# beast-dev/beast-mcmc

Measured on NVIDIA H100. Metric: tree log-likelihood evals/sec, higher is better.
Workload: dtype f64

## Files before the change

beast-mcmc_b200/csrc/api.cu:

```cuda
#include "../../include/libhmsbeagle_b200.h"
#include "engine.h"
#include "multi.h"

#include <algorithm>
#include <atomic>
#include <chrono>
#include <cmath>
#include <cstdio>
#include <cstdlib>
#include <cstring>
#include <string>
#include <unordered_map>

using namespace b200;

namespace {

std::mutex gMutex;
std::vector<Instance*> gInstances;

const long kSupportedFlags =
    BEAGLE_FLAG_PRECISION_DOUBLE | BEAGLE_FLAG_PRECISION_SINGLE | BEAGLE_FLAG_COMPUTATION_SYNCH | BEAGLE_FLAG_EIGEN_REAL |
    BEAGLE_FLAG_EIGEN_COMPLEX | BEAGLE_FLAG_SCALING_MANUAL | BEAGLE_FLAG_SCALING_DYNAMIC |
    BEAGLE_FLAG_SCALERS_RAW | BEAGLE_FLAG_SCALERS_LOG | BEAGLE_FLAG_VECTOR_NONE | BEAGLE_FLAG_THREADING_NONE |
    BEAGLE_FLAG_PROCESSOR_GPU | BEAGLE_FLAG_FRAMEWORK_CUDA | BEAGLE_FLAG_PARALLELOPS_GRID |
    BEAGLE_FLAG_PREORDER_TRANSPOSE_AUTO;

int envInt(const char* name, int dflt) {
    const char* v = getenv(name);
    return v ? atoi(v) : dflt;
}

int flushPending(Instance* in);

Instance* getInstance(int id) {
    std::lock_guard<std::mutex> lock(gMutex);
    if (id < 0 || id >= (int)gInstances.size()) return nullptr;
    return gInstances[id];
}

#define SH(id, expr)                                                                         \
    do {                                                                                     \
        Instance* p__ = getInstance(id);                                                     \
        if (p__ != nullptr && p__->shard != nullptr) {                                       \
            Sharded* sh = static_cast<Sharded*>(p__->shard);                                 \
            (void)sh;                                                                        \
            return (expr);                                                                   \
        }                                                                                    \
    } while (0)

#define GET_INSTANCE_LAZY(in, id)                                       \
    Instance* in = getInstance(id);                                     \
    if (in == nullptr) return BEAGLE_ERROR_UNINITIALIZED_INSTANCE;      \
    if (in->shard != nullptr) return BEAGLE_ERROR_NO_IMPLEMENTATION;    \
    if (cudaSetDevice(in->device) != cudaSuccess) return BEAGLE_ERROR_GENERAL;

#define GET_INSTANCE(in, id)                                            \
    GET_INSTANCE_LAZY(in, id)                                           \
    if (!in->pendingMats.empty() || !in->pendingOps.empty()) {          \
        const int flushRc__ = flushPending(in);                         \
        if (flushRc__ != BEAGLE_SUCCESS) return flushRc__;              \
    }

#define CUDA_OK(expr)                                                                        \
    do {                                                                                     \
        cudaError_t e__ = (expr);                                                            \
        if (e__ != cudaSuccess) {                                                            \
            if (getenv("B200_BEAGLE_DEBUG"))                                                 \
                fprintf(stderr, "[b200-beagle] %s failed: %s (%s:%d)\n", #expr,              \
                        cudaGetErrorString(e__), __FILE__, __LINE__);                        \
            return e__ == cudaErrorMemoryAllocation ? BEAGLE_ERROR_OUT_OF_MEMORY             \
                                                    : BEAGLE_ERROR_GENERAL;                  \
        }                                                                                    \
    } while (0)

struct TimedScope {
    Instance* in;
    int cls;
    cudaEvent_t a = nullptr, b = nullptr;
    TimedScope(Instance* i, int c, int kernels = 1) : in(i), cls(c) {
        if (in->timing) {
            in->timedLaunches[cls] += kernels - 1;
            cudaEventCreate(&a);
            cudaEventCreate(&b);
            cudaEventRecord(a, in->stream);
        }
    }
    ~TimedScope() {
        if (in->timing) {
            cudaEventRecord(b, in->stream);
            in->timed[cls].push_back({a, b});
        }
    }
};

void* stage(Instance* in, const void* src, size_t bytes) {
    size_t need = (bytes + 255) & ~size_t(255);
    if (need > in->stageSize) return nullptr;
    if (in->stagePos + need > in->stageSize) {
        cudaStreamSynchronize(in->stream);
        in->stagePos = 0;
    }
    char* h = in->hStage + in->stagePos;
    char* d = in->dStage + in->stagePos;
    memcpy(h, src, bytes);
    if (cudaMemcpyAsync(d, h, bytes, cudaMemcpyHostToDevice, in->stream) != cudaSuccess) return nullptr;
    in->stagePos += need;
    return d;
}

int uploadSmall(Instance* in, void* dDst, const void* src, size_t bytes) {
    size_t need = (bytes + 255) & ~size_t(255);
    if (need > in->stageSize) return BEAGLE_ERROR_OUT_OF_RANGE;
    if (in->stagePos + need > in->stageSize) {
        cudaStreamSynchronize(in->stream);
        in->stagePos = 0;
    }
    char* h = in->hStage + in->stagePos;
    memcpy(h, src, bytes);
    in->stagePos += need;
    CUDA_OK(cudaMemcpyAsync(dDst, h, bytes, cudaMemcpyHostToDevice, in->stream));
    return BEAGLE_SUCCESS;
}

char* ensurePartials(Instance* in, int idx) {
    if (in->partials[idx] == nullptr) {
        if (in->nextSlot >= in->nSlots) return nullptr;
        in->slotOf[idx] = in->nextSlot++;
        in->partials[idx] = in->partialsBase + (size_t)in->slotOf[idx] * in->partialsElems * in->elemBytes();
    }
    return in->partials[idx];
}

bool validRange(int idx, int n) { return idx >= 0 && idx < n; }

void destroyInstance(Instance* in) {
    if (in->shard != nullptr) { shardedDestroy(in); delete in; return; }
    cudaSetDevice(in->device);
    exchangeRelease(in);
    if (in->stream) cudaStreamSynchronize(in->stream);
    cudaFree(in->partialsBase); cudaFree(in->states8Base); cudaFree(in->states32Base);
    for (CachedPlan& cp : in->planCache) { cp.dropGraph(); cudaFree(cp.dBlock); }
    cudaFree(in->dEigen); cudaFree(in->dMat); cudaFree(in->dEvec); cudaFree(in->dIncSums); cudaFree(in->dIncCounter);
    cudaFree(in->dRecipe);
    if (in->hMapped) cudaFreeHost(in->hMapped); cudaFree(in->dRates); cudaFree(in->dWeights);
    cudaFree(in->dFreqs); cudaFree(in->dScale); cudaFree(in->dPatternWeights);
    cudaFree(in->dPatternPartitions); cudaFree(in->dSite); cudaFree(in->dBlockSums); cudaFree(in->dOut);
    cudaFree(in->dCounter); cudaFree(in->dStage); cudaFree(in->dScratch);
    if (in->hStage) cudaFreeHost(in->hStage);
    if (in->hOut) cudaFreeHost(in->hOut);
    for (int c = 0; c < T_CLASSES; ++c)
        for (auto& ev : in->timed[c]) { cudaEventDestroy(ev.first); cudaEventDestroy(ev.second); }
    if (in->stream) cudaStreamDestroy(in->stream);
    delete in;
}

std::vector<BeagleResource> gResources;
std::vector<int> gShardDevices;
int gShardResource = -1;
std::vector<std::string> gResourceStrings;
BeagleResourceList gResourceList = {nullptr, 0};
std::once_flag gResourceOnce;

void buildResources() {
    int n = 0;
    if (cudaGetDeviceCount(&n) != cudaSuccess) { cudaGetLastError(); n = 0; }
    gResourceStrings.reserve(2 * (n + 1));
    gResourceStrings.push_back("CPU (host)");
    gResourceStrings.push_back("no host implementation in this library | use a GPU resource (1..N)");
    for (int d = 0; d < n; ++d) {
        cudaDeviceProp prop;
        if (cudaGetDeviceProperties(&prop, d) != cudaSuccess) { cudaGetLastError(); continue; }
        char buf[512];
        snprintf(buf, sizeof buf, "%s", prop.name);
        gResourceStrings.push_back(buf);
        snprintf(buf, sizeof buf, "Global memory (MB): %zu | SMs: %d | compute capability: %d.%d | "
                 "native walk kernels (sm_90a), fp64 arithmetic, fp64 or fp32 (4-state) partials",
                 (size_t)(prop.totalGlobalMem >> 20), prop.multiProcessorCount, prop.major, prop.minor);
        gResourceStrings.push_back(buf);
    }
    gShardDevices.clear();
    if (const char* env = getenv("B200_SHARD_DEVICES")) {
        for (const char* q = env; *q;) {
            char* end = nullptr;
            const long d = strtol(q, &end, 10);
            if (end == q) break;
            if (d >= 0 && d < n) gShardDevices.push_back((int)d);
            q = (*end == ',') ? end + 1 : end;
        }
    } else {
        for (int d = 0; d < n; ++d) gShardDevices.push_back(d);
    }
    if (gShardDevices.size() > (size_t)kMaxGroup) gShardDevices.resize(kMaxGroup);
    if (!gShardDevices.empty()) {
        char buf[512];
        snprintf(buf, sizeof buf, "GPU x %zu (pattern-sharded)", gShardDevices.size());
        gResourceStrings.push_back(buf);
        snprintf(buf, sizeof buf, "one instance over %zu GPUs | contiguous pattern blocks (Patterns.java:142-169 rule) | "
                 "per-shard sums added over NVLink inside the root kernel", gShardDevices.size());
        gResourceStrings.push_back(buf);
        gShardResource = (int)(gResourceStrings.size() / 2) - 1;
    }
    size_t count = gResourceStrings.size() / 2;
    gResources.resize(count);
    for (size_t r = 0; r < count; ++r) {
        gResources[r].name = const_cast<char*>(gResourceStrings[2 * r].c_str());
        gResources[r].description = const_cast<char*>(gResourceStrings[2 * r + 1].c_str());
        gResources[r].supportFlags = (r == 0) ? (BEAGLE_FLAG_PROCESSOR_CPU | BEAGLE_FLAG_FRAMEWORK_CPU) : kSupportedFlags;
        gResources[r].requiredFlags = (r == 0) ? BEAGLE_FLAG_FRAMEWORK_CPU : BEAGLE_FLAG_FRAMEWORK_CUDA;
    }
    gResourceList.list = gResources.data();
    gResourceList.length = (int)count;
}

char gImplName[] = "B200-CUDA-Double";
char gImplNameSingle[] = "B200-CUDA-Single";
char gImplDesc[] = "sm_90a walk kernels: one launch per operation list, shared-memory operand stack";


struct Sub { int begin, end, pBase, pLimit; };
struct Plan {
    std::vector<int> order;
    std::vector<Sub> subs;
    std::vector<int> phaseStart;
};

void planPhases(const std::vector<HostOp>& ops, int nBuffers, bool allowReorder, int fixedT, int wantSubs, int minT,
                int smallRemainder, Plan& plan) {
    const int n = (int)ops.size();
    auto single = [&]() {
        plan.order.resize(n);
        for (int k = 0; k < n; ++k) plan.order[k] = k;
        plan.subs.assign(1, Sub{0, n, 0, 0});
        plan.phaseStart = {0, 1};
    };
    if (!allowReorder || n < 2) { single(); return; }
    std::vector<int> writer(nBuffers, -1);
    for (int k = 0; k < n; ++k) {
        if (writer[ops[k].dest] >= 0) { single(); return; }
        writer[ops[k].dest] = k;
    }
    std::vector<int> ch0(n, -1), ch1(n, -1), parent(n, -1);
    for (int k = 0; k < n; ++k) {
        const int a = writer[ops[k].c1], b = writer[ops[k].c2];
        if (a >= 0) { if (a >= k || parent[a] >= 0) { single(); return; } ch0[k] = a; parent[a] = k; }
        if (b >= 0 && ops[k].c2 != ops[k].c1) { if (b >= k || parent[b] >= 0) { single(); return; } ch1[k] = b; parent[b] = k; }
        if (ops[k].dest == ops[k].c1 || ops[k].dest == ops[k].c2) { single(); return; }
    }
    std::vector<char> alive(n, 1);
    std::vector<int> size(n), need(n);
    std::vector<std::pair<int, int>> stack;
    plan.order.clear(); plan.order.reserve(n);
    plan.subs.clear(); plan.phaseStart.assign(1, 0);
    int remaining = n;
    while (remaining > 0) {
        const int T = fixedT > 0 ? fixedT : (remaining <= smallRemainder ? remaining : std::max(minT, (remaining + wantSubs - 1) / wantSubs));
        for (int k = 0; k < n; ++k) {
            if (!alive[k]) continue;
            const int a = (ch0[k] >= 0 && alive[ch0[k]]) ? ch0[k] : -1;
            const int b = (ch1[k] >= 0 && alive[ch1[k]]) ? ch1[k] : -1;
            size[k] = 1 + (a >= 0 ? size[a] : 0) + (b >= 0 ? size[b] : 0);
            int na = a >= 0 ? need[a] : 0, nb = b >= 0 ? need[b] : 0;
            if (na < nb) std::swap(na, nb);
            need[k] = std::max(1, std::max(na, nb + (nb > 0 ? 1 : 0)));
        }
        for (int r = 0; r < n; ++r) {
            if (!alive[r] || size[r] > T) continue;
            if (parent[r] >= 0 && size[parent[r]] <= T) continue;
            const int begin = (int)plan.order.size();
            stack.push_back({r, 0});
            while (!stack.empty()) {
                auto [k, stageNo] = stack.back();
                stack.pop_back();
                if (stageNo == 1) { plan.order.push_back(k); continue; }
                stack.push_back({k, 1});
                const int a = (ch0[k] >= 0 && alive[ch0[k]]) ? ch0[k] : -1;
                const int b = (ch1[k] >= 0 && alive[ch1[k]]) ? ch1[k] : -1;
                const int na = a >= 0 ? need[a] : -1, nb = b >= 0 ? need[b] : -1;
                if (na >= nb) { if (b >= 0) stack.push_back({b, 0}); if (a >= 0) stack.push_back({a, 0}); }
                else          { if (a >= 0) stack.push_back({a, 0}); if (b >= 0) stack.push_back({b, 0}); }
            }
            plan.subs.push_back(Sub{begin, (int)plan.order.size(), 0, 0});
        }
        for (int q = plan.subs[plan.phaseStart.back()].begin; q < (int)plan.order.size(); ++q) alive[plan.order[q]] = 0;
        std::stable_sort(plan.subs.begin() + plan.phaseStart.back(), plan.subs.end(),
                         [](const Sub& a, const Sub& b) { return (a.end - a.begin) > (b.end - b.begin); });
        remaining = n - (int)plan.order.size();
        plan.phaseStart.push_back((int)plan.subs.size());
    }
}

void planLevels(const std::vector<HostOp>& ops, int nBuffers, Plan& plan) {
    const int n = (int)ops.size();
    std::vector<int> writer(nBuffers, -1), level(n, 0);
    bool hazard = false;
    for (int k = 0; k < n; ++k) { if (writer[ops[k].dest] >= 0) hazard = true; writer[ops[k].dest] = k; }
    int maxLevel = 0;
    for (int k = 0; k < n && !hazard; ++k) {
        for (int src : {ops[k].c1, ops[k].c2}) {
            const int w = writer[src];
            if (w < 0) continue;
            if (w >= k) { hazard = true; break; }
            level[k] = std::max(level[k], level[w] + 1);
        }
        maxLevel = std::max(maxLevel, level[k]);
    }
    plan.order.resize(n);
    for (int k = 0; k < n; ++k) plan.order[k] = k;
    plan.subs.clear();
    if (hazard) { plan.subs.assign(1, Sub{0, n, 0, 0}); plan.phaseStart = {0, 1}; return; }
    std::stable_sort(plan.order.begin(), plan.order.end(), [&](int a, int b) { return level[a] < level[b]; });
    plan.phaseStart.assign(1, 0);
    for (int pos = 0; pos < n; ++pos) {
        if (pos > 0 && level[plan.order[pos]] != level[plan.order[pos - 1]]) plan.phaseStart.push_back((int)plan.subs.size());
        plan.subs.push_back(Sub{pos, pos + 1, 0, 0});
    }
    plan.phaseStart.push_back((int)plan.subs.size());
}

void planPreorderPhases(const std::vector<HostOp>& ops, int nBuffers, int fixedT, int wantSubs, int minT,
                        int smallRemainder, Plan& plan) {
    const int n = (int)ops.size();
    std::vector<int> writer(nBuffers, -1), parent(n, -1);
    bool ok = n >= 2;
    for (int k = 0; k < n && ok; ++k) { ok = writer[ops[k].dest] < 0; writer[ops[k].dest] = k; }
    for (int k = 0; k < n && ok; ++k) {
        const int a = writer[ops[k].c1];
        ok = writer[ops[k].c2] < 0 && (a < 0 || a < k) && ops[k].dest != ops[k].c1 && ops[k].dest != ops[k].c2;
        parent[k] = a;
    }
    if (!ok) { planLevels(ops, nBuffers, plan); return; }
    std::vector<std::vector<int>> kids(n);
    for (int k = 0; k < n; ++k) if (parent[k] >= 0) kids[parent[k]].push_back(k);
    std::vector<char> alive(n, 1);
    std::vector<int> size(n), stack;
    std::vector<std::vector<int>> phases;
    int remaining = n;
    while (remaining > 0) {
        const int T = fixedT > 0 ? fixedT : (remaining <= smallRemainder ? remaining : std::max(minT, (remaining + wantSubs - 1) / wantSubs));
        for (int k = n - 1; k >= 0; --k) {
            if (!alive[k]) continue;
            size[k] = 1;
            for (int c : kids[k]) if (alive[c]) size[k] += size[c];
        }
        std::vector<int> roots;
        for (int r = 0; r < n; ++r)
            if (alive[r] && size[r] <= T && !(parent[r] >= 0 && alive[parent[r]] && size[parent[r]] <= T)) roots.push_back(r);
        for (int r : roots) {
            stack.assign(1, r);
            while (!stack.empty()) {
                const int k = stack.back(); stack.pop_back();
                if (!alive[k]) continue;
                alive[k] = 0; --remaining;
                for (int c : kids[k]) if (alive[c]) stack.push_back(c);
            }
        }
        phases.push_back(std::move(roots));
    }
    std::vector<int> phaseOf(n, -1), rootOf(n, -1);
    for (int ph = 0; ph < (int)phases.size(); ++ph)
        for (int r : phases[ph]) { phaseOf[r] = ph; rootOf[r] = r; }
    for (int k = 0; k < n; ++k)
        if (rootOf[k] < 0) { rootOf[k] = rootOf[parent[k]]; phaseOf[k] = phaseOf[parent[k]]; }
    plan.order.clear(); plan.order.reserve(n);
    plan.subs.clear(); plan.phaseStart.assign(1, 0);
    for (int ph = (int)phases.size() - 1; ph >= 0; --ph) {
        for (int r : phases[ph]) {
            const int begin = (int)plan.order.size();
            stack.assign(1, r);
            while (!stack.empty()) {
                const int k = stack.back(); stack.pop_back();
                plan.order.push_back(k);
                for (int q = (int)kids[k].size() - 1; q >= 0; --q)
                    if (rootOf[kids[k][q]] == r) stack.push_back(kids[k][q]);
            }
            plan.subs.push_back(Sub{begin, (int)plan.order.size(), 0, 0});
        }
        std::stable_sort(plan.subs.begin() + plan.phaseStart.back(), plan.subs.end(),
                         [](const Sub& a, const Sub& b) { return (a.end - a.begin) > (b.end - b.begin); });
        plan.phaseStart.push_back((int)plan.subs.size());
    }
}

cudaError_t launchPlan(Instance* in, const void* dOps, const void* dSubs, const std::vector<int>& phaseStart,
                       const std::vector<int>& phaseDepth, bool fourPath, int maxWindow, bool preOrder, int eigenSlot = -1,
                       bool aligned = false, const void* dSnap = nullptr, int nSnap = 0, const void* dVirtTips = nullptr) {
    const bool virt = dVirtTips != nullptr;
    cudaError_t e = cudaSuccess;
    if (nSnap > 0) {
        TimedScope ts(in, T_PARTIALS);
        e = launchCherrySnapshot(in, static_cast<const int4*>(dSnap), nSnap);
    }
    for (size_t ph = 0; ph + 1 < phaseStart.size() && e == cudaSuccess; ++ph) {
        const int s0 = phaseStart[ph], s1 = phaseStart[ph + 1];
        if (s1 <= s0) continue;
        TimedScope ts(in, T_PARTIALS);
        if (fourPath && eigenSlot >= 0 && !preOrder && (ph >= phaseDepth.size() || phaseDepth[ph] == 0)) {
            e = launchWalk4E(in, static_cast<const Op4*>(dOps), static_cast<const int4*>(dSubs) + s0, s1 - s0, maxWindow,
                             aligned, in->hEigen.data() + (size_t)eigenSlot * 36, static_cast<const int4*>(dVirtTips));
            continue;
        }
        if (virt) return cudaErrorInvalidValue;
        e = fourPath ? launchWalk4(in, static_cast<const Op4*>(dOps), static_cast<const int4*>(dSubs) + s0, s1 - s0,
                                   ph < phaseDepth.size() ? phaseDepth[ph] : 0, maxWindow, preOrder)
                     : launchWalkGeneric(in, static_cast<const DevOp*>(dOps), static_cast<const int4*>(dSubs) + s0, s1 - s0,
                                         maxWindow, preOrder);
    }
    return e;
}

cudaError_t accumulateInList(Instance* in, const std::vector<CumGroup>& groups) {
    for (const CumGroup& g : groups) {
        int* dIdx = static_cast<int*>(stage(in, g.indices.data(), sizeof(int) * g.indices.size()));
        if (dIdx == nullptr) return cudaErrorMemoryAllocation;
        cudaError_t e = launchScaleAccumulate(in, dIdx, (int)g.indices.size(), in->dScale + (size_t)g.cum * in->Ppad, 1.0,
                                              g.pBegin, g.pEnd);
        if (e != cudaSuccess) return e;
        in->scaleIsLog[g.cum] = 1;
    }
    return cudaSuccess;
}

void noteScaleWrites(Instance* in, const std::vector<HostOp>& hops) {
    for (const HostOp& o : hops) if (o.sw >= 0) in->scaleIsLog[o.sw] = in->logScalers ? 1 : 0;
}


cudaError_t storeCherries(Instance* in, const int* bufs, int count) {
    if (in->cherryTip1.empty()) return cudaSuccess;
    std::vector<int4> items;
    for (int k = 0; k < count; ++k) {
        const int b = bufs[k];
        if (!validRange(b, in->nBuffers) || in->cherryTip1[b] < 0 || in->cherryStored[b]) continue;
        items.push_back(make_int4(in->slotOf[b], b, in->cherryTip1[b], in->cherryTip2[b]));
        in->cherryStored[b] = 1;
    }
    if (items.empty()) return cudaSuccess;
    const int4* dItems = static_cast<const int4*>(stage(in, items.data(), sizeof(int4) * items.size()));
    cudaError_t e = cudaErrorMemoryAllocation;
    if (dItems != nullptr) {
        TimedScope ts(in, T_PARTIALS);
        e = launchCherryStore(in, dItems, (int)items.size());
    }
    if (e != cudaSuccess) for (const int4& it : items) in->cherryStored[it.y] = 0;
    return e;
}

cudaError_t storeExternal(Instance* in, const std::vector<CherryRef>& external) {
    std::vector<int> bufs;
    for (const CherryRef& x : external) if (x.tip1 < 0) bufs.push_back(x.buf);
    return storeCherries(in, bufs.data(), (int)bufs.size());
}

cudaError_t settleCherriesOf(Instance* in, int t) {
    std::vector<int> deps;
    for (int b = 0; b < (int)in->cherryTip1.size(); ++b)
        if (in->cherryTip1[b] >= 0 && (in->cherryTip1[b] == t || in->cherryTip2[b] == t)) deps.push_back(b);
    const cudaError_t e = storeCherries(in, deps.data(), (int)deps.size());
    if (e == cudaSuccess) for (int b : deps) in->cherryTip1[b] = -1;
    return e;
}

void noteCherryWrites(Instance* in, const std::vector<HostOp>& hops, const std::vector<CherryRef>& cherries) {
    if (in->cherryTip1.empty()) return;
    for (const HostOp& o : hops) in->cherryTip1[o.dest] = -1;
    for (const CherryRef& c : cherries) {
        in->cherryTip1[c.buf] = c.tip1; in->cherryTip2[c.buf] = c.tip2; in->cherryStored[c.buf] = 0;
    }
}

int prepareOps(Instance* in, const std::vector<HostOp>& hops, bool byPartition) {
    for (const HostOp& o : hops) {
        if (!validRange(o.dest, in->nBuffers) || !validRange(o.c1, in->nBuffers) ||
            !validRange(o.c2, in->nBuffers) || !validRange(o.m1, in->nMatrices) ||
            !validRange(o.m2, in->nMatrices))
            return BEAGLE_ERROR_OUT_OF_RANGE;
        if (o.sw != BEAGLE_OP_NONE && !validRange(o.sw, in->nScale)) return BEAGLE_ERROR_OUT_OF_RANGE;
        if (o.sr != BEAGLE_OP_NONE && !validRange(o.sr, in->nScale)) return BEAGLE_ERROR_OUT_OF_RANGE;
        if (o.cum != BEAGLE_OP_NONE && !validRange(o.cum, in->nScale)) return BEAGLE_ERROR_OUT_OF_RANGE;
        if (byPartition && !validRange(o.part, in->partitionCount)) return BEAGLE_ERROR_OUT_OF_RANGE;
    }
    {
        std::vector<char> written(in->nBuffers, 0);
        for (const HostOp& o : hops) written[o.dest] = 1;
        auto holdsData = [&](int b) { return written[b] || in->partials[b] != nullptr || in->states32[b] != nullptr; };
        for (const HostOp& o : hops) {
            if (!holdsData(o.c1) || !holdsData(o.c2)) return BEAGLE_ERROR_OUT_OF_RANGE;
            if (o.kind == 1 && !written[o.c1] && in->states32[o.c1] != nullptr) return BEAGLE_ERROR_OUT_OF_RANGE;
        }
    }
    for (const HostOp& o : hops) {
        if (ensurePartials(in, o.dest) == nullptr) return BEAGLE_ERROR_OUT_OF_MEMORY;
        if (in->states32[o.dest] != nullptr) in->bufferEpoch++;
        in->states8[o.dest] = nullptr;
        in->states32[o.dest] = nullptr;
    }
    return BEAGLE_SUCCESS;
}

int eigenFormSlot(const Instance* in, const std::vector<HostOp>& hops) {
    if (!in->eigenWalk || in->matCP == 0 || in->walkVariant != 0 || hops.empty() || hops[0].kind == 1) return -1;
    const int E = in->matEigen[hops[0].m1];
    if (E < 0 || !in->eigenReal[E]) return -1;
    const unsigned gen = in->eigenGen[E];
    for (const HostOp& o : hops)
        if (in->matEigen[o.m1] != E || in->matEigen[o.m2] != E || in->matEigenGen[o.m1] != gen || in->matEigenGen[o.m2] != gen)
            return -1;
    return E;
}

int planAndLaunch(Instance* in, const std::vector<HostOp>& hops, bool byPartition) {
    const int n = (int)hops.size();
    if (n == 0) return BEAGLE_SUCCESS;
    static_assert(sizeof(HostOp) == 10 * sizeof(int), "HostOp is compared bytewise");
    if (in->planCacheSize > 0) {
        for (CachedPlan& cp : in->planCache) {
            if (cp.dBlock == nullptr || cp.n != n || cp.byPartition != byPartition || cp.epoch != in->bufferEpoch ||
                memcmp(cp.key.data(), hops.data(), sizeof(HostOp) * (size_t)n) != 0)
                continue;
            const int eigenSlot = cp.fourPath ? eigenFormSlot(in, hops) : -1;
            bool stale = cp.readsVirtual && eigenSlot < 0;
            for (const CherryRef& x : cp.external)
                stale = stale || (x.tip1 >= 0 && (in->cherryTip1[x.buf] != x.tip1 || in->cherryTip2[x.buf] != x.tip2));
            if (stale) { cp.dropGraph(); cp.n = -1; continue; }
            CUDA_OK(storeExternal(in, cp.external));
            cp.lastUse = ++in->planClock;
            cp.hits++;
            const unsigned eigenGenNow = eigenSlot >= 0 ? in->eigenGen[eigenSlot] : 0u;
            const void* dSnap = static_cast<char*>(cp.dBlock) + cp.snapOffset;
            const int nSnap = (int)cp.cherries.size();
            const void* dTips = cp.readsVirtual ? static_cast<char*>(cp.dBlock) + cp.tipsOffset : nullptr;
            if (cp.graphExec != nullptr && (cp.graphEigen != eigenSlot || cp.graphEigenGen != eigenGenNow)) {
                if (cp.graphAllEigen && eigenSlot >= 0 && cp.graphEigen == eigenSlot &&
                    updateWalk4EGraph(cp.graphExec, cp.graphKernelNodes, in->hEigen.data() + (size_t)eigenSlot * 36) == cudaSuccess) {
                    cp.graphEigenGen = eigenGenNow;
                } else {
                    cudaGetLastError();
                    cp.dropGraph();
                    cp.hits = 1;
                    if (++cp.graphInvalidations >= 4) cp.graphFailed = true;
                }
            }
            int launches = nSnap > 0;
            for (size_t ph = 0; ph + 1 < cp.phaseStart.size(); ++ph) launches += cp.phaseStart[ph + 1] > cp.phaseStart[ph];
            if (in->useGraphs && launches >= 2 && cp.cumGroups.empty()) {
                if (cp.graphExec == nullptr && !cp.graphFailed && cp.hits >= 2 && !in->timing &&
                    cudaStreamBeginCapture(in->stream, cudaStreamCaptureModeThreadLocal) == cudaSuccess) {
                    const cudaError_t e1 = launchPlan(in, cp.dBlock, static_cast<char*>(cp.dBlock) + cp.subsOffset, cp.phaseStart,
                                                      cp.phaseDepth, cp.fourPath, cp.maxWindow, cp.preOrder, eigenSlot,
                                                      !cp.byPartition, dSnap, nSnap, dTips);
                    cp.graphEigen = eigenSlot;
                    cp.graphEigenGen = eigenGenNow;
                    cudaGraph_t g = nullptr;
                    const cudaError_t e2 = cudaStreamEndCapture(in->stream, &g);
                    if (e1 != cudaSuccess || e2 != cudaSuccess || g == nullptr ||
                        cudaGraphInstantiate(&cp.graphExec, g, 0) != cudaSuccess) {
                        cp.graphExec = nullptr;
                        cp.graphFailed = true;
                        if (g) cudaGraphDestroy(g);
                    } else {
                        cp.graph = g;
                        cp.graphKernelNodes.clear();
                        cp.graphAllEigen = cp.fourPath && eigenSlot >= 0 && !cp.preOrder;
                        for (int dpt : cp.phaseDepth) cp.graphAllEigen = cp.graphAllEigen && dpt == 0;
                        size_t nn = 0;
                        if (cudaGraphGetNodes(g, nullptr, &nn) == cudaSuccess && nn > 0) {
                            std::vector<cudaGraphNode_t> nodes(nn);
                            cudaGraphNodeType ty;
                            if (cudaGraphGetNodes(g, nodes.data(), &nn) == cudaSuccess)
                                for (size_t q = 0; q < nn; ++q)
                                    if (cudaGraphNodeGetType(nodes[q], &ty) == cudaSuccess && ty == cudaGraphNodeTypeKernel)
                                        cp.graphKernelNodes.push_back(nodes[q]);
                        }
                        if (cp.graphKernelNodes.empty()) cp.graphAllEigen = false;
                    }
                    if (getenv("B200_BEAGLE_DEBUG"))
                        fprintf(stderr, "[b200-beagle] graph %s: %d launches\n", cp.graphExec ? "captured" : "capture failed",
                                launches);
                    cudaGetLastError();
                }
                if (cp.graphExec != nullptr) {
                    TimedScope ts(in, T_PARTIALS, launches);
                    CUDA_OK(cudaGraphLaunch(cp.graphExec, in->stream));
                    noteScaleWrites(in, hops);
                    noteCherryWrites(in, hops, cp.cherries);
                    return BEAGLE_SUCCESS;
                }
            }
            CUDA_OK(launchPlan(in, cp.dBlock, static_cast<char*>(cp.dBlock) + cp.subsOffset, cp.phaseStart, cp.phaseDepth,
                               cp.fourPath, cp.maxWindow, cp.preOrder, eigenSlot, !cp.byPartition, dSnap, nSnap,
                               dTips));
            CUDA_OK(accumulateInList(in, cp.cumGroups));
            noteScaleWrites(in, hops);
            noteCherryWrites(in, hops, cp.cherries);
            return BEAGLE_SUCCESS;
        }
    }
    {
        const int rcPrepare = prepareOps(in, hops, byPartition);
        if (rcPrepare != BEAGLE_SUCCESS) return rcPrepare;
    }
    const bool fourState = in->matCP > 0;
    const bool preOrder = hops[0].kind == 1;
    const int eigenSlot = fourState ? eigenFormSlot(in, hops) : -1;
    std::vector<char> written(in->nBuffers, 0);
    std::vector<int> firstWrite(in->nBuffers, n);
    for (int k = n - 1; k >= 0; --k) { written[hops[k].dest] = 1; firstWrite[hops[k].dest] = k; }
    std::vector<CherryRef> cherries;
    std::vector<int4> snap;
    std::vector<HostOp> kept;
    bool readsVirtual = false;
    if (!in->cherryTip1.empty() && !byPartition && !preOrder && eigenSlot >= 0 && !in->stackTail) {
        std::vector<int> writes(in->nBuffers, 0), firstRead(in->nBuffers, n);
        for (int k = 0; k < n; ++k) {
            writes[hops[k].dest]++;
            firstRead[hops[k].c1] = std::min(firstRead[hops[k].c1], k);
            firstRead[hops[k].c2] = std::min(firstRead[hops[k].c2], k);
        }
        for (int k = 0; k < n; ++k) {
            const HostOp& o = hops[k];
            if (in->states8[o.c1] != nullptr && in->states8[o.c2] != nullptr && o.sw == BEAGLE_OP_NONE &&
                o.sr == BEAGLE_OP_NONE && o.cum == BEAGLE_OP_NONE && writes[o.dest] == 1 && firstRead[o.dest] > k) {
                cherries.push_back(CherryRef{o.dest, o.c1, o.c2});
                snap.push_back(make_int4(o.dest, o.m1, o.m2, 0));
            } else {
                kept.push_back(o);
            }
        }
        if (kept.empty()) { cherries.clear(); snap.clear(); }
        readsVirtual = !cherries.empty();
        for (const HostOp& o : hops)
            for (int c : {o.c1, o.c2})
                readsVirtual = readsVirtual || (!written[c] && in->states32[c] == nullptr && in->cherryTip1[c] >= 0);
    }
    Plan plan;
    int maxWindow = in->Ppad;
    const int patsPerWarp = !fourState ? 16 : (in->walkVariant == 2 ? 8 * in->tensorR : (32 / in->matCP) * in->walkR);
    const int warpsPerSM = fourState ? 32 : 12;
    auto wantSubsFor = [&](int window) {
        const int warpsPerSub = std::max(1, (window + patsPerWarp - 1) / patsPerWarp);
        const int over = in->phaseOversub > 0 ? in->phaseOversub : (warpsPerSub >= 32 ? 1 : 2);
        return std::max(1, over * ((in->smCount * warpsPerSM + warpsPerSub - 1) / warpsPerSub));
    };
    if (!byPartition && !preOrder) {
        planPhases(cherries.empty() ? hops : kept, in->nBuffers, in->reorder != 0, in->phaseT, wantSubsFor(in->Ppad),
                   in->phaseTmin, in->phaseSmall, plan);
        bool served = true;
        for (size_t ph = 0; readsVirtual && ph + 1 < plan.phaseStart.size(); ++ph) {
            const int nSubs = plan.phaseStart[ph + 1] - plan.phaseStart[ph];
            served = served && (nSubs == 0 || walk4pServes(in, nSubs, in->Ppad));
        }
        if (!served) {
            readsVirtual = false;
            if (!cherries.empty()) {
                cherries.clear(); snap.clear(); kept.clear();
                planPhases(hops, in->nBuffers, in->reorder != 0, in->phaseT, wantSubsFor(in->Ppad), in->phaseTmin,
                           in->phaseSmall, plan);
            }
        }
        for (Sub& sb : plan.subs) { sb.pBase = 0; sb.pLimit = in->Ppad; }
    }
    const std::vector<HostOp>& L = cherries.empty() ? hops : kept;
    const int nL = (int)L.size();
    std::vector<int> vt1(readsVirtual ? in->nBuffers : 0, -1), vt2(readsVirtual ? in->nBuffers : 0, -1);
    for (const CherryRef& c : cherries) { vt1[c.buf] = c.tip1; vt2[c.buf] = c.tip2; }
    std::vector<CherryRef> external;
    {
        std::vector<char> seen(in->nBuffers, 0);
        for (int k = 0; k < n; ++k)
            for (int c : {hops[k].c1, hops[k].c2}) {
                if (firstWrite[c] < k || in->states32[c] != nullptr || seen[c]) continue;
                seen[c] = 1;
                const bool virt = readsVirtual && !written[c] && in->cherryTip1[c] >= 0;
                external.push_back(CherryRef{c, virt ? in->cherryTip1[c] : -1, virt ? in->cherryTip2[c] : -1});
                if (virt) { vt1[c] = in->cherryTip1[c]; vt2[c] = in->cherryTip2[c]; }
            }
    }
    CUDA_OK(storeExternal(in, external));
    {
        if (!byPartition) {
            if (preOrder) {
                if (in->prePhases) planPreorderPhases(hops, in->nBuffers, in->phaseT, wantSubsFor(in->Ppad), in->phaseTmin, in->phaseSmall, plan);
                else planLevels(hops, in->nBuffers, plan);
                for (Sub& sb : plan.subs) { sb.pBase = 0; sb.pLimit = in->Ppad; }
            }
        } else {
            std::vector<std::vector<int>> members(in->partitionCount);
            for (int k = 0; k < n; ++k) members[hops[k].part].push_back(k);
            std::vector<Plan> plans;
            std::vector<int> base;
            maxWindow = 1;
            for (int part = 0; part < in->partitionCount; ++part) {
                if (members[part].empty()) continue;
                std::vector<HostOp> sub(members[part].size());
                for (size_t q = 0; q < sub.size(); ++q) sub[q] = hops[members[part][q]];
                Plan pl;
                const int window = in->partEnd[part] - in->partBegin[part];
                if (sub[0].kind == 1 && in->prePhases) planPreorderPhases(sub, in->nBuffers, in->phaseT, wantSubsFor(std::max(1, window)), in->phaseTmin, in->phaseSmall, pl);
                else if (sub[0].kind == 1) planLevels(sub, in->nBuffers, pl);
                else planPhases(sub, in->nBuffers, in->reorder != 0, in->phaseT, wantSubsFor(std::max(1, window)), in->phaseTmin, in->phaseSmall, pl);
                base.push_back((int)plan.order.size());
                for (int idx : pl.order) plan.order.push_back(members[part][idx]);
                for (Sub& sb : pl.subs) {
                    sb.begin += base.back(); sb.end += base.back();
                    sb.pBase = in->partBegin[part]; sb.pLimit = in->partEnd[part];
                }
                maxWindow = std::max(maxWindow, window);
                plans.push_back(std::move(pl));
            }
            plan.phaseStart.assign(1, 0);
            for (size_t ph = 0;; ++ph) {
                bool any = false;
                for (const Plan& pl : plans) {
                    if (ph + 1 >= pl.phaseStart.size()) continue;
                    any = true;
                    for (int q = pl.phaseStart[ph]; q < pl.phaseStart[ph + 1]; ++q) plan.subs.push_back(pl.subs[q]);
                }
                if (!any) break;
                plan.phaseStart.push_back((int)plan.subs.size());
            }
        }
    }
    const std::vector<int>& order = plan.order;

    const bool stackEverywhere = fourState && in->walkVariant == 1 && !preOrder;
    const bool stackThin = fourState && in->walkVariant == 0 && in->stackTail && !preOrder;
    const int maxDepth = (stackEverywhere || stackThin) ? in->stackDepthMax : 0;
    const int nPhases = (int)plan.phaseStart.size() - 1;
// ... 208 lines not shown
        if (slot->capacity < blockBytes) {
            if (slot->dBlock) cudaFree(slot->dBlock);
            slot->dBlock = nullptr; slot->capacity = 0;
            if (cudaMalloc(&slot->dBlock, blockBytes) == cudaSuccess) slot->capacity = blockBytes; else cudaGetLastError();
        }
        if (slot->dBlock != nullptr &&
            cudaMemcpyAsync(slot->dBlock, dOps, blockBytes, cudaMemcpyDeviceToDevice, in->stream) == cudaSuccess) {
            slot->key = hops; slot->n = n; slot->byPartition = byPartition; slot->epoch = in->bufferEpoch;
            slot->subsOffset = subsOffset; slot->snapOffset = snapOffset; slot->tipsOffset = tipsOffset;
            slot->cherries = cherries; slot->external = external; slot->readsVirtual = readsVirtual;
            slot->phaseStart = plan.phaseStart; slot->phaseDepth = depths;
            slot->fourPath = fourPath; slot->maxWindow = maxWindow; slot->preOrder = preOrder;
            slot->lastUse = ++in->planClock;
            slot->cumGroups = cumGroups;
            slot->graphFailed = !cumGroups.empty();
        } else if (slot->dBlock != nullptr) {
            slot->n = -1;
        }
    }
    if (tmp != nullptr) { cudaStreamSynchronize(in->stream); cudaFree(tmp); }
    CUDA_OK(e);
    return BEAGLE_SUCCESS;
}

}

namespace b200 {
Instance* instanceById(int id) { return getInstance(id); }
}

extern "C" {

#ifndef B200_SOURCE_HASH
#define B200_SOURCE_HASH "unhashed"
#endif
const char* beagleGetVersion(void) { return "4.0.1-b200+" B200_SOURCE_HASH; }
const char* b200GetSourceHash(void) { return B200_SOURCE_HASH; }

const char* beagleGetCitation(void) {
    return "H100-native tree-likelihood engine exposing the BEAGLE API.\n"
           "API after: Ayres et al. (2019) BEAGLE 3. Syst Biol 68:1052-1061.";
}

BeagleResourceList* beagleGetResourceList(void) {
    std::call_once(gResourceOnce, buildResources);
    return &gResourceList;
}

BeagleBenchmarkedResourceList* beagleGetBenchmarkedResourceList(
    int tipCount, int compactBufferCount, int stateCount, int patternCount, int categoryCount, int* resourceList,
    int resourceCount, long preferenceFlags, long requirementFlags, int eigenModelCount, int partitionCount,
    int calculateDerivatives, long benchmarkFlags);

int beagleCreateInstance(int tipCount, int partialsBufferCount, int compactBufferCount, int stateCount,
                         int patternCount, int eigenBufferCount, int matrixBufferCount, int categoryCount,
                         int scaleBufferCount, int* resourceList, int resourceCount, long preferenceFlags,
                         long requirementFlags, BeagleInstanceDetails* returnInfo) {
    if (tipCount < 0 || partialsBufferCount < 0 || compactBufferCount < 0 || stateCount < 2 ||
        patternCount < 1 || eigenBufferCount < 0 || matrixBufferCount < 0 || categoryCount < 1 ||
        scaleBufferCount < 0 || stateCount > 255)
        return BEAGLE_ERROR_OUT_OF_RANGE;
    if (requirementFlags & ~kSupportedFlags) return BEAGLE_ERROR_NO_RESOURCE;
    const bool singleFits = stateCount <= 4 && categoryCount <= 8;
    if (requirementFlags & BEAGLE_FLAG_PRECISION_SINGLE) {
        if (!singleFits || (requirementFlags & BEAGLE_FLAG_PRECISION_DOUBLE)) return BEAGLE_ERROR_NO_RESOURCE;
    }
    const bool single = singleFits && ((requirementFlags & BEAGLE_FLAG_PRECISION_SINGLE) ||
                                       ((preferenceFlags & BEAGLE_FLAG_PRECISION_SINGLE) &&
                                        !((preferenceFlags | requirementFlags) & BEAGLE_FLAG_PRECISION_DOUBLE)));
    BeagleResourceList* rl = beagleGetResourceList();
    int resource = -1;
    if (resourceList == nullptr || resourceCount <= 0) {
        if (rl->length > 1) resource = 1;
    } else {
        for (int k = 0; k < resourceCount; ++k)
            if (resourceList[k] >= 1 && resourceList[k] < rl->length) { resource = resourceList[k]; break; }
    }
    if (resource < 1) return BEAGLE_ERROR_NO_RESOURCE;

    if (resource == gShardResource) {
        Instance* parent = new Instance();
        parent->resource = resource;
        parent->device = gShardDevices[0];
        parent->P = patternCount; parent->S = stateCount; parent->C = categoryCount; parent->tipCount = tipCount;
        const int g = (int)gShardDevices.size();
        const int rc = shardedCreate(parent, g, gShardDevices.data(), tipCount, partialsBufferCount, compactBufferCount,
                                     stateCount, patternCount, eigenBufferCount, matrixBufferCount, categoryCount,
                                     scaleBufferCount, preferenceFlags, requirementFlags, returnInfo);
        if (rc != BEAGLE_SUCCESS) { delete parent; return rc; }
        if (returnInfo != nullptr) {
            returnInfo->resourceNumber = resource;
            returnInfo->resourceName = rl->list[resource].name;
            parent->flags = returnInfo->flags;
        }
        std::lock_guard<std::mutex> lock(gMutex);
        int id = -1;
        for (size_t k = 0; k < gInstances.size(); ++k) if (gInstances[k] == nullptr) { id = (int)k; break; }
        if (id < 0) { gInstances.push_back(nullptr); id = (int)gInstances.size() - 1; }
        gInstances[id] = parent;
        parent->id = id;
        return id;
    }

    Instance* in = new Instance();
    in->device = resource - 1;
    in->resource = resource;
    if (cudaSetDevice(in->device) != cudaSuccess) { delete in; return BEAGLE_ERROR_NO_RESOURCE; }
    in->tipCount = tipCount; in->nPartials = partialsBufferCount; in->nCompact = compactBufferCount;
    in->S = stateCount; in->P = patternCount; in->nEigen = eigenBufferCount; in->nMatrices = matrixBufferCount;
    in->C = categoryCount; in->nScale = scaleBufferCount;
    in->Sp = stateCount <= 4 ? 4 : ((stateCount + 7) / 8) * 8;
    in->Ppad = ((patternCount + 31) / 32) * 32;
    in->nBuffers = partialsBufferCount + compactBufferCount;
    in->nSets = std::max(1, eigenBufferCount);
    in->single = single;
    in->complexEigen = (requirementFlags | preferenceFlags) & BEAGLE_FLAG_EIGEN_COMPLEX;
    in->logScalers = (requirementFlags | preferenceFlags) & BEAGLE_FLAG_SCALERS_LOG;
    in->flags = (single ? BEAGLE_FLAG_PRECISION_SINGLE : BEAGLE_FLAG_PRECISION_DOUBLE) | BEAGLE_FLAG_COMPUTATION_SYNCH |
                BEAGLE_FLAG_SCALING_MANUAL |
                BEAGLE_FLAG_VECTOR_NONE | BEAGLE_FLAG_THREADING_NONE | BEAGLE_FLAG_PROCESSOR_GPU |
                BEAGLE_FLAG_FRAMEWORK_CUDA | BEAGLE_FLAG_PARALLELOPS_GRID |
                (in->complexEigen ? BEAGLE_FLAG_EIGEN_COMPLEX : BEAGLE_FLAG_EIGEN_REAL) |
                (in->logScalers ? BEAGLE_FLAG_SCALERS_LOG : BEAGLE_FLAG_SCALERS_RAW);
    if ((requirementFlags | preferenceFlags) & BEAGLE_FLAG_PREORDER_TRANSPOSE_AUTO) in->flags |= BEAGLE_FLAG_PREORDER_TRANSPOSE_AUTO;
    if ((requirementFlags | preferenceFlags) & BEAGLE_FLAG_SCALING_DYNAMIC) {
        in->flags &= ~BEAGLE_FLAG_SCALING_MANUAL;
        in->flags |= BEAGLE_FLAG_SCALING_DYNAMIC;
    }
    in->partialsElems = (size_t)in->C * in->Ppad * in->Sp;
    if (in->Sp == 4 && in->C <= 32) {
        int cp = 1;
        while (cp < in->C) cp <<= 1;
        in->matCP = cp;
        in->matStride = (size_t)16 * cp + 52 * (size_t)in->C;
        in->matStride = (in->matStride + 3) & ~size_t(3);
    } else {
        in->matCP = 0;
        in->matStride = (size_t)in->C * in->Sp * (in->Sp + 2 * (size_t)(in->Sp + 4));
    }
    in->slotOf.assign(in->nBuffers, -1);
    in->partials.assign(in->nBuffers, nullptr);
    in->states8.assign(in->nBuffers, nullptr);
    in->states32.assign(in->nBuffers, nullptr);
    in->scaleIsLog.assign(std::max(1, in->nScale), in->logScalers ? 1 : 0);
    in->matEigen.assign(std::max(1, in->nMatrices), -1);
    in->matEigenGen.assign(std::max(1, in->nMatrices), 0u);
    in->eigenGen.assign(std::max(1, in->nEigen), 0u);
    in->eigenReal.assign(std::max(1, in->nEigen), 0);
    in->hEigen.assign((size_t)std::max(1, in->nEigen) * 36, 0.0);
    in->eigenWalk = envInt("B200_EIGEN_WALK", 1);
    in->tipMode = envInt("B200_TIP_MODE", 3);
    in->thinTipMode = envInt("B200_THIN_TIP_MODE", in->tipMode);
    in->virtualCherries = envInt("B200_VIRTUAL_CHERRIES", 1);
    in->walkBlock = 128;
    in->walkVariant = envInt("B200_WALK_VARIANT", 0);
    in->reorder = envInt("B200_REORDER", 1);
    in->forward = envInt("B200_FORWARD", 1);
    in->lookahead = envInt("B200_LOOKAHEAD", 1);
    in->useGraphs = envInt("B200_GRAPHS", 1);
    in->prePhases = envInt("B200_PRE_PHASES", 1);
    in->lookaheadPre = envInt("B200_LOOKAHEAD_PRE", 1);
    in->planCacheSize = std::max(0, std::min(16, envInt("B200_PLAN_CACHE", 4)));
    in->planCache.reserve(16);
    in->thinR1 = envInt("B200_THIN_R1", 1);
    in->stackTail = envInt("B200_STACK_TAIL", 0);
    in->phaseT = envInt("B200_PHASE_T", 0);
    in->phaseTmin = std::max(1, envInt("B200_PHASE_TMIN", 4));
    in->phaseSmall = envInt("B200_PHASE_SMALL", 24);
    in->phaseOversub = std::max(0, envInt("B200_PHASE_OVERSUB", 0));
    in->walkMinBlocks = envInt("B200_WALK_MINB", 4);
    in->walkMinBlocksSet = getenv("B200_WALK_MINB") != nullptr;
    in->tensorR = envInt("B200_TENSOR_R", 2) >= 4 ? 4 : 2;
    in->genericMma = envInt("B200_GENERIC_MMA", 1);
    in->mmaWarps = envInt("B200_MMA_WARPS", 4) == 8 ? 8 : 4;
    cudaDeviceProp prop;
    bool ok = cudaGetDeviceProperties(&prop, in->device) == cudaSuccess;
    if (ok) { in->smCount = prop.multiProcessorCount; in->maxSmemOptin = prop.sharedMemPerBlockOptin; }
    in->walkR = envInt("B200_WALK_R", 4);
    if (in->walkR != 1 && in->walkR != 2 && in->walkR != 4 && in->walkR != 8) in->walkR = 4;
    if (getenv("B200_WALK_R") == nullptr && in->matCP > 0) {
        const int G = 32 / in->matCP;
        while (in->walkR > 1 && (in->Ppad + G * in->walkR - 1) / (G * in->walkR) < in->smCount) in->walkR >>= 1;
    }
    in->stackDepthMax = std::min(64, std::max(0, envInt("B200_STACK_DEPTH", 12)));
    if (single) { in->walkVariant = 0; in->stackTail = 0; }

    ok = ok && cudaStreamCreateWithFlags(&in->stream, cudaStreamNonBlocking) == cudaSuccess;
    const size_t eigenStride = 2 * (size_t)in->S * in->S + 2 * in->S;
    const size_t matElems = (size_t)in->nMatrices * in->matStride;
    const int rootBlocks = (in->Ppad + 255) / 256;
    in->stageSize = size_t(8) << 20;
    auto alloc = [&](auto** p, size_t elems) {
        if (!ok) return;
        using T = std::remove_pointer_t<std::remove_pointer_t<decltype(p)>>;
        size_t bytes = std::max<size_t>(elems, 1) * sizeof(T);
        ok = cudaMalloc(reinterpret_cast<void**>(p), bytes) == cudaSuccess &&
             cudaMemsetAsync(*p, 0, bytes, in->stream) == cudaSuccess;
    };
    alloc(&in->dEigen, std::max(1, in->nEigen) * eigenStride);
    alloc(&in->dMat, matElems);
    if (in->matCP > 0) alloc(&in->dEvec, (size_t)in->nMatrices * in->matCP * 4);
    if (in->matCP > 0 && in->matCP <= 8 && in->virtualCherries) {
        alloc(&in->dRecipe, (size_t)in->nBuffers * 32 * in->matCP);
        in->cherryTip1.assign(in->nBuffers, -1);
        in->cherryTip2.assign(in->nBuffers, -1);
        in->cherryStored.assign(in->nBuffers, 0);
    }
    if (in->matCP > 0 && in->matCP <= 8) {
        alloc(&in->dIncSums, (size_t)in->Ppad / 4 + 8);
        alloc(&in->dIncCounter, 4);
        in->fuseSmall = envInt("B200_FUSE", 1);
        if (ok && in->fuseSmall) {
            if (cudaHostAlloc(reinterpret_cast<void**>(&in->hMapped), 64, cudaHostAllocMapped) == cudaSuccess &&
                cudaHostGetDevicePointer(reinterpret_cast<void**>(&in->dMapped), in->hMapped, 0) == cudaSuccess) {
                memset(in->hMapped, 0, 64);
            } else {
                cudaGetLastError();
                if (in->hMapped) cudaFreeHost(in->hMapped);
                in->hMapped = nullptr;
            }
        }
    }
    alloc(&in->dRates, (size_t)in->nSets * in->C);
    alloc(&in->dWeights, (size_t)in->nSets * in->C);
    alloc(&in->dFreqs, (size_t)in->nSets * in->Sp);
    alloc(&in->dScale, (size_t)in->nScale * in->Ppad);
    alloc(&in->dPatternWeights, in->Ppad);
    alloc(&in->dPatternPartitions, in->Ppad);
    alloc(&in->dSite, in->Ppad);
    alloc(&in->dBlockSums, rootBlocks);
    alloc(&in->dOut, 1024);
    alloc(&in->dCounter, 4);
    alloc(&in->dStage, in->stageSize);
    alloc(&in->states8Base, (size_t)std::max(1, in->tipCount) * in->Ppad);
    alloc(&in->states32Base, (size_t)std::max(1, in->tipCount) * in->Ppad);
    if (ok) {
        int want[2] = {in->nPartials, std::max(1, in->nPartials - std::min(in->nCompact, in->tipCount))};
        for (int attempt = 0; attempt < 2 && in->partialsBase == nullptr; ++attempt) {
            size_t bytes = (size_t)want[attempt] * in->partialsElems * in->elemBytes();
            if (cudaMalloc(reinterpret_cast<void**>(&in->partialsBase), bytes) == cudaSuccess) in->nSlots = want[attempt];
            else { cudaGetLastError(); in->partialsBase = nullptr; }
        }
        if (in->partialsBase == nullptr) { destroyInstance(in); return BEAGLE_ERROR_OUT_OF_MEMORY; }
    }
    ok = ok && cudaMallocHost(reinterpret_cast<void**>(&in->hStage), in->stageSize) == cudaSuccess;
    ok = ok && cudaMallocHost(reinterpret_cast<void**>(&in->hOut), 1024 * sizeof(double)) == cudaSuccess;
    if (ok) {
        in->hRates.assign((size_t)in->nSets * in->C, 1.0);
        in->hWeights.assign((size_t)in->nSets * in->C, 0.0);
        in->hFreqs.assign((size_t)in->nSets * 4, 0.0);
        std::vector<double> ones((size_t)std::max(in->nSets * in->C, in->Ppad), 1.0);
        ok = cudaMemcpyAsync(in->dRates, ones.data(), sizeof(double) * in->nSets * in->C, cudaMemcpyHostToDevice,
                             in->stream) == cudaSuccess;
        std::vector<double> w(in->Ppad, 0.0);
        std::fill(w.begin(), w.begin() + in->P, 1.0);
        ok = ok && cudaMemcpyAsync(in->dPatternWeights, w.data(), sizeof(double) * in->Ppad, cudaMemcpyHostToDevice,
                                   in->stream) == cudaSuccess;
        ok = ok && cudaStreamSynchronize(in->stream) == cudaSuccess;
    }
    if (!ok) {
        cudaError_t e = cudaGetLastError();
        destroyInstance(in);
        return e == cudaErrorMemoryAllocation ? BEAGLE_ERROR_OUT_OF_MEMORY : BEAGLE_ERROR_GENERAL;
    }
    in->partitionCount = 1;
    in->partBegin.assign(1, 0);
    in->partEnd.assign(1, in->P);
    {
        std::lock_guard<std::mutex> lock(gMutex);
        int id = -1;
        for (size_t k = 0; k < gInstances.size(); ++k) if (gInstances[k] == nullptr) { id = (int)k; break; }
        if (id < 0) { gInstances.push_back(nullptr); id = (int)gInstances.size() - 1; }
        gInstances[id] = in;
        in->id = id;
    }
    if (returnInfo != nullptr) {
        returnInfo->resourceNumber = resource;
        returnInfo->resourceName = rl->list[resource].name;
        returnInfo->implName = single ? gImplNameSingle : gImplName;
        returnInfo->implDescription = gImplDesc;
        returnInfo->flags = in->flags;
    }
    return in->id;
}

int beagleFinalizeInstance(int instance) {
    Instance* in = nullptr;
    {
        std::lock_guard<std::mutex> lock(gMutex);
        if (instance < 0 || instance >= (int)gInstances.size() || gInstances[instance] == nullptr)
            return BEAGLE_ERROR_UNINITIALIZED_INSTANCE;
        in = gInstances[instance];
        gInstances[instance] = nullptr;
    }
    destroyInstance(in);
    return BEAGLE_SUCCESS;
}

int beagleFinalize(void) {
    std::vector<Instance*> all;
    {
        std::lock_guard<std::mutex> lock(gMutex);
        all.swap(gInstances);
    }
    for (Instance* in : all) if (in) destroyInstance(in);
    return BEAGLE_SUCCESS;
}

int beagleSetCPUThreadCount(int instance, int) {
    SH(instance, BEAGLE_SUCCESS);
    GET_INSTANCE(in, instance);
    (void)in;
    return BEAGLE_SUCCESS;
}

int beagleSetTipStates(int instance, int tipIndex, const int* inStates) {
    SH(instance, shSetTipStates(sh, tipIndex, inStates));
    GET_INSTANCE(in, instance);
    if (!validRange(tipIndex, in->nBuffers) || inStates == nullptr) return BEAGLE_ERROR_OUT_OF_RANGE;
    std::vector<int> s32(in->Ppad, in->S);
    std::vector<uint8_t> s8(in->Ppad, (uint8_t)in->S);
    for (int p = 0; p < in->P; ++p) {
        int s = inStates[p];
        if (s < 0 || s >= in->S) s = in->S;
        s32[p] = s;
        s8[p] = (uint8_t)s;
    }
    if (tipIndex >= in->tipCount) return BEAGLE_ERROR_OUT_OF_RANGE;
    CUDA_OK(settleCherriesOf(in, tipIndex));
    in->states32[tipIndex] = in->states32Base + (size_t)tipIndex * in->Ppad;
    in->states8[tipIndex] = in->states8Base + (size_t)tipIndex * in->Ppad;
    CUDA_OK(cudaMemcpyAsync(in->states32[tipIndex], s32.data(), sizeof(int) * in->Ppad, cudaMemcpyHostToDevice, in->stream));
    CUDA_OK(cudaMemcpyAsync(in->states8[tipIndex], s8.data(), in->Ppad, cudaMemcpyHostToDevice, in->stream));
    CUDA_OK(cudaStreamSynchronize(in->stream));
    in->bufferEpoch++;
    return BEAGLE_SUCCESS;
}

int beagleGetTipStates(int instance, int tipIndex, int* outStates) {
    SH(instance, shGetTipStates(sh, tipIndex, outStates));
    GET_INSTANCE(in, instance);
    if (!validRange(tipIndex, in->nBuffers) || in->states32[tipIndex] == nullptr) return BEAGLE_ERROR_OUT_OF_RANGE;
    CUDA_OK(cudaMemcpyAsync(outStates, in->states32[tipIndex], sizeof(int) * in->P, cudaMemcpyDeviceToHost, in->stream));
    CUDA_OK(cudaStreamSynchronize(in->stream));
    return BEAGLE_SUCCESS;
}

static int setPartialsImpl(Instance* in, int bufferIndex, const double* inPartials, bool perCategory) {
    if (!validRange(bufferIndex, in->nBuffers) || inPartials == nullptr) return BEAGLE_ERROR_OUT_OF_RANGE;
    char* dst = ensurePartials(in, bufferIndex);
    if (dst == nullptr) return BEAGLE_ERROR_OUT_OF_MEMORY;
    CUDA_OK(settleCherriesOf(in, bufferIndex));
    if (!in->cherryTip1.empty()) in->cherryTip1[bufferIndex] = -1;
    std::vector<double> tmp(in->partialsElems, 0.0);
    for (int c = 0; c < in->C; ++c)
        for (int p = 0; p < in->Ppad; ++p) {
            double* row = tmp.data() + ((size_t)c * in->Ppad + p) * in->Sp;
            if (p < in->P) {
                const double* src = inPartials + ((size_t)(perCategory ? c : 0) * in->P + p) * in->S;
// ... 78 lines not shown
int beagleSetEigenDecomposition(int instance, int eigenIndex, const double* inEigenVectors,
                                const double* inInverseEigenVectors, const double* inEigenValues) {
    SH(instance, shBroadcast(sh, [&](int c) { return beagleSetEigenDecomposition(c, eigenIndex, inEigenVectors, inInverseEigenVectors, inEigenValues); }));
    GET_INSTANCE(in, instance);
    if (!validRange(eigenIndex, in->nEigen)) return BEAGLE_ERROR_OUT_OF_RANGE;
    const size_t S = in->S, stride = 2 * S * S + 2 * S;
    std::vector<double> pack(stride, 0.0);
    memcpy(pack.data(), inEigenVectors, sizeof(double) * S * S);
    memcpy(pack.data() + S * S, inInverseEigenVectors, sizeof(double) * S * S);
    memcpy(pack.data() + 2 * S * S, inEigenValues, sizeof(double) * (in->complexEigen ? 2 * S : S));
    if (in->matCP > 0) {
        double h[36] = {0.0};
        for (size_t k = 0; k < S; ++k) h[32 + k] = inEigenValues[k];
        for (size_t i = 0; i < S; ++i)
            for (size_t k = 0; k < S; ++k) { h[4 * i + k] = inEigenVectors[i * S + k]; h[16 + 4 * i + k] = inInverseEigenVectors[i * S + k]; }
        bool real = true;
        if (in->complexEigen) for (size_t k = 0; k < S; ++k) real = real && inEigenValues[S + k] == 0.0;
        double* dst = in->hEigen.data() + (size_t)eigenIndex * 36;
        if (memcmp(dst, h, sizeof h) != 0 || in->eigenGen[eigenIndex] == 0 || (bool)in->eigenReal[eigenIndex] != real) {
            memcpy(dst, h, sizeof h);
            in->eigenGen[eigenIndex]++;
        }
        in->eigenReal[eigenIndex] = real ? 1 : 0;
    }
    return uploadSmall(in, in->dEigen + (size_t)eigenIndex * stride, pack.data(), sizeof(double) * stride);
}

int beagleSetStateFrequencies(int instance, int stateFrequenciesIndex, const double* inStateFrequencies) {
    SH(instance, shBroadcast(sh, [&](int c) { return beagleSetStateFrequencies(c, stateFrequenciesIndex, inStateFrequencies); }));
    GET_INSTANCE(in, instance);
    if (!validRange(stateFrequenciesIndex, in->nSets)) return BEAGLE_ERROR_OUT_OF_RANGE;
    std::vector<double> f(in->Sp, 0.0);
    memcpy(f.data(), inStateFrequencies, sizeof(double) * in->S);
    if (in->hFreqs.size() == (size_t)in->nSets * 4 && in->S <= 4)
        for (int i = 0; i < 4; ++i) in->hFreqs[(size_t)stateFrequenciesIndex * 4 + i] = i < in->S ? inStateFrequencies[i] : 0.0;
    return uploadSmall(in, in->dFreqs + (size_t)stateFrequenciesIndex * in->Sp, f.data(), sizeof(double) * in->Sp);
}

int beagleSetCategoryWeights(int instance, int categoryWeightsIndex, const double* inCategoryWeights) {
    SH(instance, shBroadcast(sh, [&](int c) { return beagleSetCategoryWeights(c, categoryWeightsIndex, inCategoryWeights); }));
    GET_INSTANCE(in, instance);
    if (!validRange(categoryWeightsIndex, in->nSets)) return BEAGLE_ERROR_OUT_OF_RANGE;
    std::copy(inCategoryWeights, inCategoryWeights + in->C, in->hWeights.begin() + (size_t)categoryWeightsIndex * in->C);
    return uploadSmall(in, in->dWeights + (size_t)categoryWeightsIndex * in->C, inCategoryWeights, sizeof(double) * in->C);
}

int beagleSetCategoryRatesWithIndex(int instance, int categoryRatesIndex, const double* inCategoryRates) {
    SH(instance, shBroadcast(sh, [&](int c) { return beagleSetCategoryRatesWithIndex(c, categoryRatesIndex, inCategoryRates); }));
    GET_INSTANCE(in, instance);
    if (!validRange(categoryRatesIndex, in->nSets)) return BEAGLE_ERROR_OUT_OF_RANGE;
    std::copy(inCategoryRates, inCategoryRates + in->C, in->hRates.begin() + (size_t)categoryRatesIndex * in->C);
    return uploadSmall(in, in->dRates + (size_t)categoryRatesIndex * in->C, inCategoryRates, sizeof(double) * in->C);
}

int beagleSetCategoryRates(int instance, const double* inCategoryRates) {
    return beagleSetCategoryRatesWithIndex(instance, 0, inCategoryRates);
}

int beagleSetPatternWeights(int instance, const double* inPatternWeights) {
    SH(instance, shSetPatternWeights(sh, inPatternWeights));
    GET_INSTANCE(in, instance);
    std::vector<double> w(in->Ppad, 0.0);
    memcpy(w.data(), inPatternWeights, sizeof(double) * in->P);
    CUDA_OK(cudaMemcpyAsync(in->dPatternWeights, w.data(), sizeof(double) * in->Ppad, cudaMemcpyHostToDevice, in->stream));
    CUDA_OK(cudaStreamSynchronize(in->stream));
    return BEAGLE_SUCCESS;
}

int beagleSetPatternPartitions(int instance, int partitionCount, const int* inPatternPartitions) {
    SH(instance, BEAGLE_ERROR_NO_IMPLEMENTATION);
    GET_INSTANCE(in, instance);
    if (partitionCount < 1 || partitionCount > 1000) return BEAGLE_ERROR_OUT_OF_RANGE;
    std::vector<int> begin(partitionCount, 0), end(partitionCount, 0);
    int prev = -1;
    for (int p = 0; p < in->P; ++p) {
        int k = inPatternPartitions[p];
        if (k < 0 || k >= partitionCount) return BEAGLE_ERROR_OUT_OF_RANGE;
        if (k < prev) return BEAGLE_ERROR_NO_IMPLEMENTATION;
        if (k != prev) { for (int q = prev + 1; q <= k; ++q) begin[q] = end[q] = p; prev = k; }
        end[k] = p + 1;
    }
    for (int q = prev + 1; q < partitionCount; ++q) begin[q] = end[q] = in->P;
    in->bufferEpoch++;
    in->partitionCount = partitionCount;
    in->partBegin = begin;
    in->partEnd = end;
    in->hostPartitions.assign(inPatternPartitions, inPatternPartitions + in->P);
    return BEAGLE_SUCCESS;
}

static int updateMatricesImpl(Instance* in, const int* eigenIndices, int eigenIndexScalar, const int* rateSets,
                              const int* probabilityIndices, const double* edgeLengths, int count) {
    if (count <= 0) return BEAGLE_SUCCESS;
    std::vector<double> block((size_t)count + (3 * (size_t)count + 1) / 2);
    int* pack = reinterpret_cast<int*>(block.data() + count);
    for (int k = 0; k < count; ++k) {
        int e = eigenIndices ? eigenIndices[k] : eigenIndexScalar;
        int r = rateSets ? rateSets[k] : 0;
        if (!validRange(probabilityIndices[k], in->nMatrices) || !validRange(e, in->nEigen) ||
            !validRange(r, in->nSets))
            return BEAGLE_ERROR_OUT_OF_RANGE;
        pack[k] = probabilityIndices[k];
        pack[count + k] = e;
        pack[2 * (size_t)count + k] = r;
    }
    if (in->matCP > 0)
        for (int k = 0; k < count; ++k) {
            const int e = eigenIndices ? eigenIndices[k] : eigenIndexScalar;
            in->matEigen[probabilityIndices[k]] = e;
            in->matEigenGen[probabilityIndices[k]] = in->eigenGen[e];
        }
    memcpy(block.data(), edgeLengths, sizeof(double) * count);
    double* dLen = static_cast<double*>(stage(in, block.data(), sizeof(double) * block.size()));
    if (dLen == nullptr) return BEAGLE_ERROR_OUT_OF_MEMORY;
    int* dIdx = reinterpret_cast<int*>(dLen + count);
    TimedScope ts(in, T_MATRICES);
    CUDA_OK(launchTransitionMatrices(in, dIdx, dIdx + count, dIdx + 2 * (size_t)count, dLen, count));
    return BEAGLE_SUCCESS;
}

}
namespace {
int flushPendingImpl(Instance* in) {
    int rc = BEAGLE_SUCCESS;
    if (!in->pendingMats.empty()) {
        const int n = (int)in->pendingMats.size();
        std::vector<int> eig(n), rate(n), prob(n);
        std::vector<double> len(n);
        for (int k = 0; k < n; ++k) {
            eig[k] = in->pendingMats[k].eigen; rate[k] = in->pendingMats[k].rateSet;
            prob[k] = in->pendingMats[k].prob; len[k] = in->pendingMats[k].len;
        }
        in->pendingMats.clear();
        rc = updateMatricesImpl(in, eig.data(), 0, rate.data(), prob.data(), len.data(), n);
    }
    if (!in->pendingOps.empty()) {
        std::vector<HostOp> hops;
        hops.swap(in->pendingOps);
        const int rc2 = planAndLaunch(in, hops, false);
        if (rc == BEAGLE_SUCCESS) rc = rc2;
    }
    return rc;
}

bool fusionPossible(const Instance* in) {
    return in->fuseSmall && in->matCP > 0 && in->matCP <= 8 && !in->timing && !in->exchangeOn && in->walkVariant == 0 &&
           in->eigenWalk && in->hMapped != nullptr;
}

int launchFused(Instance* in, int E, int wIdx, int fIdx, int cum, double* outSum) {
    IncArgs A;
    memset(&A, 0, sizeof A);
    A.partials = in->partialsBase; A.stride = in->partialsElems; A.states = in->states8Base; A.mats = in->dMat;
    A.evecs = in->dEvec; A.scale = in->dScale; A.matStride = in->matStride;
    A.S = in->S; A.C = in->C; A.Ppad = in->Ppad; A.P = in->P; A.logScalers = in->logScalers ? 1 : 0;
    const double* h = in->hEigen.data() + (size_t)E * 36;
    for (int q = 0; q < 16; ++q) { A.V[q] = h[q]; A.Vi[q] = h[16 + q]; }
    for (int q = 0; q < 4; ++q) A.eval[q] = h[32 + q];
    A.nMats = (int)in->pendingMats.size();
    std::unordered_map<int, int> pendingOf;
    for (int q = 0; q < A.nMats; ++q) {
        A.mat[q] = IncMat{in->pendingMats[q].prob, in->pendingMats[q].rateSet, in->pendingMats[q].len};
        for (int c = 0; c < 8; ++c) A.rate[q][c] = c < in->C ? in->hRates[(size_t)in->pendingMats[q].rateSet * in->C + c] : 0.0;
        pendingOf[in->pendingMats[q].prob] = q;
    }
    A.nOps = (int)in->pendingOps.size();
    {
        std::vector<int> outside;
        for (int k = 0; k < A.nOps; ++k)
            for (int c : {in->pendingOps[k].c1, in->pendingOps[k].c2}) {
                bool written = false;
                for (int w = 0; w < k; ++w) written = written || in->pendingOps[w].dest == c;
                if (!written) outside.push_back(c);
            }
        CUDA_OK(storeCherries(in, outside.data(), (int)outside.size()));
    }
    int prevDest = -1;
    for (int k = 0; k < A.nOps; ++k) {
        const HostOp& o = in->pendingOps[k];
        IncOp& d = A.op[k];
        const bool t1 = in->states32[o.c1] != nullptr, t2 = in->states32[o.c2] != nullptr;
        int c1 = o.c1, c2 = o.c2, m1 = o.m1, m2 = o.m2;
        d.flags = 0;
        if (k > 0 && !t1 && c1 == prevDest) d.flags = 1;
        else if (k > 0 && !t2 && c2 == prevDest) { std::swap(c1, c2); std::swap(m1, m2); d.flags = 1; }
        const bool s1 = in->states32[c1] != nullptr, s2 = in->states32[c2] != nullptr;
        d.dest = in->slotOf[o.dest];
        d.c1 = s1 ? -(c1 + 1) : in->slotOf[c1];
        d.c2 = s2 ? -(c2 + 1) : in->slotOf[c2];
        auto mat = [&](int m) { auto it = pendingOf.find(m); return it == pendingOf.end() ? m : -(it->second + 1); };
        d.m1 = mat(m1); d.m2 = mat(m2);
        d.sw = o.sw; d.sr = o.sw >= 0 ? -1 : o.sr;
        prevDest = o.dest;
    }
    for (int c = 0; c < 8; ++c) A.weights[c] = c < in->C ? in->hWeights[(size_t)wIdx * in->C + c] : 0.0;
    for (int i = 0; i < 4; ++i) A.freqs[i] = in->hFreqs[(size_t)fIdx * 4 + i];
    A.cum = cum == BEAGLE_OP_NONE ? nullptr : in->dScale + (size_t)cum * in->Ppad;
    A.patternWeights = in->dPatternWeights; A.site = in->dSite; A.blockSums = in->dIncSums; A.counter = in->dIncCounter;
    A.out = in->dOut;
    A.hostOut = in->dMapped;
    A.hostFlag = reinterpret_cast<volatile unsigned long long*>(in->dMapped + 1);
    A.seq = ++in->incSeq;
    CUDA_OK(launchIncremental(in, A));
    noteScaleWrites(in, in->pendingOps);
    noteCherryWrites(in, in->pendingOps, {});
    in->pendingMats.clear();
    in->pendingOps.clear();
    in->fusedLaunches++;
    volatile unsigned long long* flag = reinterpret_cast<volatile unsigned long long*>(in->hMapped + 1);
    const auto t0 = std::chrono::steady_clock::now();
    long spins = 0;
    while (*flag != A.seq) {
        if ((++spins & 0xfff) == 0 &&
            std::chrono::duration<double>(std::chrono::steady_clock::now() - t0).count() > 5.0) {
            CUDA_OK(cudaStreamSynchronize(in->stream));
            if (*flag != A.seq) return BEAGLE_ERROR_GENERAL;
        }
    }
    std::atomic_thread_fence(std::memory_order_acquire);
    *outSum = in->hMapped[0];
    return std::isnan(*outSum) ? BEAGLE_ERROR_FLOATING_POINT : BEAGLE_SUCCESS;
}
int flushPending(Instance* in) { return flushPendingImpl(in); }
}
extern "C" {

int beagleUpdateTransitionMatrices(int instance, int eigenIndex, const int* probabilityIndices,
                                   const int* firstDerivativeIndices, const int* secondDerivativeIndices,
                                   const double* edgeLengths, int count) {
    SH(instance, shBroadcast(sh, [&](int c) { return beagleUpdateTransitionMatrices(c, eigenIndex, probabilityIndices, firstDerivativeIndices, secondDerivativeIndices, edgeLengths, count); }));
    GET_INSTANCE_LAZY(in, instance);
    if (firstDerivativeIndices != nullptr || secondDerivativeIndices != nullptr)
        return BEAGLE_ERROR_NO_IMPLEMENTATION;
    bool defer = fusionPossible(in) && count >= 1 && in->pendingOps.empty() &&
                 (int)in->pendingMats.size() + count <= kIncMaxMats && validRange(eigenIndex, in->nEigen) &&
                 in->eigenReal[eigenIndex] && in->eigenGen[eigenIndex] > 0;
    for (int k = 0; k < count && defer; ++k) {
        defer = validRange(probabilityIndices[k], in->nMatrices);
        for (const Instance::PendingMat& pm : in->pendingMats) defer = defer && pm.prob != probabilityIndices[k] && pm.eigen == eigenIndex;
        for (int q = 0; q < k && defer; ++q) defer = probabilityIndices[q] != probabilityIndices[k];
    }
    if (defer) {
        for (int k = 0; k < count; ++k) {
            in->pendingMats.push_back(Instance::PendingMat{probabilityIndices[k], eigenIndex, 0, edgeLengths[k]});
            in->matEigen[probabilityIndices[k]] = eigenIndex;
            in->matEigenGen[probabilityIndices[k]] = in->eigenGen[eigenIndex];
        }
        return BEAGLE_SUCCESS;
    }
    if (!in->pendingMats.empty() || !in->pendingOps.empty()) { const int rc = flushPending(in); if (rc != BEAGLE_SUCCESS) return rc; }
    return updateMatricesImpl(in, nullptr, eigenIndex, nullptr, probabilityIndices, edgeLengths, count);
}

int beagleUpdateTransitionMatricesWithMultipleModels(int instance, const int* eigenIndices,
                                                     const int* categoryRateIndices, const int* probabilityIndices,
                                                     const int* firstDerivativeIndices,
                                                     const int* secondDerivativeIndices, const double* edgeLengths,
                                                     int count) {
    SH(instance, shBroadcast(sh, [&](int c) { return beagleUpdateTransitionMatricesWithMultipleModels(c, eigenIndices, categoryRateIndices, probabilityIndices, firstDerivativeIndices, secondDerivativeIndices, edgeLengths, count); }));
    GET_INSTANCE(in, instance);
    if (firstDerivativeIndices != nullptr || secondDerivativeIndices != nullptr)
        return BEAGLE_ERROR_NO_IMPLEMENTATION;
    return updateMatricesImpl(in, eigenIndices, 0, categoryRateIndices, probabilityIndices, edgeLengths, count);
}

static inline size_t matIndex(const Instance* in, int c, int i, int j) {
    return in->matCP ? ((size_t)j * in->matCP + c) * 4 + i : ((size_t)c * in->Sp + j) * in->Sp + i;
}

int beagleSetTransitionMatrix(int instance, int matrixIndex, const double* inMatrix, double) {
    SH(instance, shBroadcast(sh, [&](int c) { return beagleSetTransitionMatrix(c, matrixIndex, inMatrix, 0.0); }));
    GET_INSTANCE(in, instance);
    if (!validRange(matrixIndex, in->nMatrices)) return BEAGLE_ERROR_OUT_OF_RANGE;
    if (in->matCP > 0) in->matEigen[matrixIndex] = -1;
    const size_t n = in->matStride;
    std::vector<double> t(n, 0.0);
    for (int c = 0; c < in->C; ++c)
        for (int i = 0; i < in->S; ++i)
            for (int j = 0; j < in->S; ++j)
            {
                const double v = inMatrix[((size_t)c * in->S + i) * in->S + j];
                t[matIndex(in, c, i, j)] = v;
                if (in->matCP) {
                    double* mm = t.data() + 16 * in->matCP;
                    mm[(size_t)c * 32 + i * 4 + j] = v;
                    double* mt = mm + (size_t)in->C * 32;
                    mt[(size_t)c * 20 + j * 4 + i] = v;
                    for (int q = 0; q < 4; ++q) {
                        if (in->S < 4) mt[(size_t)c * 20 + in->S * 4 + q] = q < in->S ? 1.0 : 0.0;
                        else mt[(size_t)c * 20 + 16 + q] = 1.0;
                    }
                } else {
                    const size_t ld = (size_t)in->Sp + 4, half = (size_t)in->C * in->Sp * in->Sp;
                    t[half + ((size_t)c * in->Sp + i) * ld + j] = v;
                    t[half + (size_t)in->C * in->Sp * ld + ((size_t)c * in->Sp + j) * ld + i] = v;
                }
            }
    CUDA_OK(cudaMemcpyAsync(in->dMat + matrixIndex * n, t.data(), sizeof(double) * n, cudaMemcpyHostToDevice, in->stream));
    CUDA_OK(cudaStreamSynchronize(in->stream));
    return BEAGLE_SUCCESS;
}

int beagleGetTransitionMatrix(int instance, int matrixIndex, double* outMatrix) {
    SH(instance, shBroadcast(sh, [&](int c) { return beagleGetTransitionMatrix(c, matrixIndex, outMatrix); }));
    GET_INSTANCE(in, instance);
    if (!validRange(matrixIndex, in->nMatrices)) return BEAGLE_ERROR_OUT_OF_RANGE;
    const size_t n = in->matStride;
// ... 677 lines not shown
```

beast-mcmc_b200/csrc/engine.h:

```cpp
#pragma once
#include <cuda_runtime.h>
#include <cstdint>
#include <mutex>
#include <vector>

namespace b200 {

struct alignas(16) DevOp {
    double* dest;
    const double* c1;
    const double* c2;
    const void* s1;
    const void* s2;
    const double* m1;
    const double* m2;
    double* scaleWrite;
    const double* scaleRead;
    double* cumScale;
    int pBegin, pEnd;
    int srcSlot1, srcSlot2;
    int dstSlot;
    int pad_;
};

struct alignas(16) Op4 {
    int dest, c1, c2, m1;
    int m2, sw, sr, cum;
    int pBegin, pEnd;
    unsigned int slots;
    int pad_;
    int pfA, pfB, pfM1, pfM2;
};

struct CherryRef { int buf, tip1, tip2; };

template <typename T> struct EdgeRefT { const T* post; const int* states; const T* pre; const double* D; double len; };
using EdgeRef = EdgeRefT<double>;

struct HostOp { int dest, sw, sr, c1, m1, c2, m2, part, cum; int kind = 0; };
struct CumGroup { int cum, pBegin, pEnd; std::vector<int> indices; };
struct CachedPlan {
    std::vector<HostOp> key;
    std::vector<CumGroup> cumGroups;
    int n = -1;
    bool byPartition = false, fourPath = false, preOrder = false;
    unsigned long epoch = 0;
    void* dBlock = nullptr;
    size_t capacity = 0, subsOffset = 0, snapOffset = 0, tipsOffset = 0;
    std::vector<CherryRef> cherries, external;
    bool readsVirtual = false;
    std::vector<int> phaseStart, phaseDepth;
    int maxWindow = 0;
    long lastUse = 0;
    long hits = 0;
    cudaGraphExec_t graphExec = nullptr;
    bool graphFailed = false;
    int graphEigen = -2;
    unsigned graphEigenGen = 0;
    int graphInvalidations = 0;
    cudaGraph_t graph = nullptr;
    std::vector<cudaGraphNode_t> graphKernelNodes;
    bool graphAllEigen = false;
    void dropGraph() {
        if (graphExec) cudaGraphExecDestroy(graphExec);
        if (graph) cudaGraphDestroy(graph);
        graphExec = nullptr; graph = nullptr; graphKernelNodes.clear(); graphAllEigen = false;
    }
};

enum TimingClass { T_PARTIALS = 0, T_MATRICES = 1, T_ROOT = 2, T_CLASSES = 3 };

constexpr int kIncMaxOps = 64, kIncMaxMats = 8;
struct IncOp { int dest, c1, c2, m1, m2, sw, sr, flags; };
struct IncMat { int prob, rateSet; double len; };
struct IncArgs {
    void* partials; size_t stride; const uint8_t* states; double* mats; double* evecs; double* scale;
    size_t matStride;
    int S, C, Ppad, P, logScalers, nOps, nMats, pad_;
    double V[16], Vi[16], eval[4];
    double weights[8], freqs[4], rate[kIncMaxMats][8];
    const double* cum; const double* patternWeights;
    double* site; double* blockSums; unsigned int* counter; double* out;
    volatile double* hostOut; volatile unsigned long long* hostFlag; unsigned long long seq;
    IncMat mat[kIncMaxMats];
    IncOp op[kIncMaxOps];
};

constexpr int kMaxGroup = 16;
struct ExchangeSlot { double value; unsigned long long seq; };
struct Exchange {
    int rank = 0, size = 1;
    unsigned long long seq = 0;
    long long timeoutCycles = 0;
    ExchangeSlot* peers[kMaxGroup] = {};
};

struct Instance {
    int id = -1, device = 0, resource = 0;
    int tipCount = 0, nPartials = 0, nCompact = 0, S = 0, P = 0, nEigen = 0, nMatrices = 0, C = 0, nScale = 0;
    int Sp = 0, Ppad = 0, nBuffers = 0, nSets = 1;
    long flags = 0;
    bool logScalers = false, complexEigen = false;
    cudaStream_t stream = nullptr;
    int smCount = 132;
    size_t maxSmemOptin = 0;

    bool single = false;
    size_t partialsElems = 0;
    size_t elemBytes() const { return single ? sizeof(float) : sizeof(double); }
    char* partialsBase = nullptr;
    int nSlots = 0, nextSlot = 0;
    std::vector<int> slotOf;
    std::vector<char*> partials;
    uint8_t* states8Base = nullptr;
    int* states32Base = nullptr;
    std::vector<uint8_t*> states8;
    std::vector<int*> states32;
    int matCP = 0;
    size_t matStride = 0;

    double* dEigen = nullptr;
    double* dMat = nullptr;
    double* dEvec = nullptr;
    std::vector<int> matEigen;
    std::vector<unsigned> matEigenGen, eigenGen;
    std::vector<char> eigenReal;
    std::vector<double> hEigen;
    int eigenWalk = 1;
    int tipMode = 2;
    int thinTipMode = 3;
    int virtualCherries = 1;
    std::vector<int> cherryTip1, cherryTip2;
    std::vector<char> cherryStored;
    double* dRecipe = nullptr;
    double* dRates = nullptr;
    std::vector<double> hRates, hWeights, hFreqs;
    double* dWeights = nullptr;
    double* dFreqs = nullptr;
    double* dScale = nullptr;
    std::vector<char> scaleIsLog;
    double* dPatternWeights = nullptr;
    int* dPatternPartitions = nullptr;
    double* dSite = nullptr;
    double* dBlockSums = nullptr;
    double* dOut = nullptr;
    unsigned int* dCounter = nullptr;
    int lookaheadPre = 1;
    int prePhases = 1;
    int useGraphs = 1;
    int lookahead = 1;
    int forward = 1;
    double* dScratch = nullptr;
    size_t scratchDoubles = 0;
    int partitionCount = 1;
    std::vector<int> partBegin, partEnd;
    std::vector<int> hostPartitions;

    char* hStage = nullptr;
    char* dStage = nullptr;
    size_t stageSize = 0, stagePos = 0;
    double* hOut = nullptr;

    int fuseSmall = 1;
    struct PendingMat { int prob, eigen, rateSet; double len; };
    std::vector<PendingMat> pendingMats;
    std::vector<HostOp> pendingOps;
    int pendingCum = -1;
    double* hMapped = nullptr;
    double* dMapped = nullptr;
    double* dIncSums = nullptr;
    unsigned int* dIncCounter = nullptr;
    unsigned long long incSeq = 0;
    long fusedLaunches = 0;

    void* shard = nullptr;
    Exchange exchange;
    ExchangeSlot* dSlots = nullptr;
    std::vector<void*> ipcOpened;
    bool exchangeOn = false;

    bool timing = false;
    std::vector<std::pair<cudaEvent_t, cudaEvent_t>> timed[T_CLASSES];
    double timedMs[T_CLASSES] = {0, 0, 0};
    long timedLaunches[T_CLASSES] = {0, 0, 0};

    size_t walkSmemConfigured = 0, genericSmemConfigured = 0, mmaSmemConfigured[8] = {0, 0, 0, 0, 0, 0, 0, 0};
    int walkBlock = 128;
    int walkVariant = 0;
    std::vector<CachedPlan> planCache;
    int planCacheSize = 4;
    long planClock = 0;
    unsigned long bufferEpoch = 0;
    int reorder = 1;
    int thinR1 = 1;
    int stackTail = 0;
    int stackDepthMax = 12;
    int walkMinBlocks = 4;
    bool walkMinBlocksSet = false;
    int mmaWarps = 4;
    int tensorR = 2;
    int genericMma = 1;
    int walkR = 4;
    int phaseTmin = 4, phaseOversub = 0, phaseSmall = 24;
    int phaseT = 0;
};

struct Sharded;
Instance* instanceById(int id);
void exchangeRelease(Instance* in);
int shardedCreate(Instance* parent, int g, const int* devices, int tipCount, int partialsBufferCount, int compactBufferCount,
                  int stateCount, int patternCount, int eigenBufferCount, int matrixBufferCount, int categoryCount,
                  int scaleBufferCount, long preferenceFlags, long requirementFlags, void* details );
void shardedDestroy(Instance* parent);

cudaError_t launchTransitionMatrices(Instance* in, const int* dProbIdx, const int* dEigenIdx,
                                     const int* dRateSet, const double* dLengths, int count);
cudaError_t launchWalk4(Instance* in, const Op4* dOps, const int4* dSubs, int nSubs, int stackDepth, int maxWindow, bool preOrder);
cudaError_t updateWalk4EGraph(cudaGraphExec_t exec, const std::vector<cudaGraphNode_t>& kernelNodes, const double* eigen);
cudaError_t launchWalk4E(Instance* in, const Op4* dOps, const int4* dSubs, int nSubs, int maxWindow, bool aligned,
                         const double* eigen, const int4* dVirtTips);
bool walk4pServes(const Instance* in, int nSubs, int maxWindow);
cudaError_t launchCherrySnapshot(Instance* in, const int4* dItems, int count);
cudaError_t launchCherryStore(Instance* in, const int4* dItems, int count);
cudaError_t launchWalkGeneric(Instance* in, const DevOp* dOps, const int4* dSubs, int nSubs, int maxWindow, bool preOrder);
size_t edgeDerivativeWorkspace(const Instance* in, int count);
cudaError_t launchEdgeDerivatives(Instance* in, const EdgeRefT<void>* dEdges, int count, const double* weights, double* outPerPattern,
                                  double* outSum, double* outSumSq, double* partial);
int compressSitePatterns(int device, int taxa, int sites, const int* hStates, int* hPatternOfSite, int* hPatterns,
                         double* hWeights, int* hPatternCount);
int crossProductBlocks(const Instance* in, int count);
cudaError_t launchCrossProducts(Instance* in, const EdgeRefT<void>* dEdges, int count, const double* rates,
                                const double* weights, double* scratch);
cudaError_t launchRoot(Instance* in, const void* root, const double* weights, const double* freqs,
                       const double* cumScale, int pBegin, int pEnd, double* dOutSlot, const Exchange* exchange = nullptr);
cudaError_t launchIncremental(Instance* in, const IncArgs& args);
cudaError_t launchCombineMatrices(Instance* in, const int* dFirst, const int* dSecond, const int* dResult, int count, bool multiply);
cudaError_t launchExchangeSum(Instance* in, const double* dVals, int n, double* dOutJoint, const Exchange* exchange);
cudaError_t launchScaleAccumulate(Instance* in, const int* dIdx, int count, double* cum, double sign,
                                  int pBegin, int pEnd);
cudaError_t launchRescalePartialsForGet(Instance* in, double* tmp, const double* cum);

}
```

beast-mcmc_b200/csrc/incr.cu:

```cuda
#include "engine.h"
#include "walk4.cuh"

namespace b200 {

namespace {

__device__ __forceinline__ double absBitsI(double v) {
    return __hiloint2double(__double2hiint(v) & 0x7fffffff, __double2loint(v));
}

template <typename T, int CP>
__device__ __forceinline__ void incrementalBody(const IncArgs& A) {
    constexpr int G = 32 / CP;
    __shared__ double sE[kIncMaxMats][CP][4];
    __shared__ __align__(16) double sP[kIncMaxMats][CP][16];
    __shared__ double red[4];
    __shared__ bool last;
    const int tid = threadIdx.x, lane = tid & 31, wib = tid >> 5;
    const int S = A.S, C = A.C;
    const int c = lane / G;
    const int p = blockIdx.x * (4 * G) + wib * G + (lane % G);
    const bool catValid = c < C;
    const int cc = catValid ? c : 0;
    const bool inRange = p < A.Ppad;
    const int pp = inRange ? p : 0;
    const size_t off0 = ((size_t)cc * A.Ppad + pp) * 4;
    for (int k = 0; k < A.nOps; ++k) {
        const IncOp op = A.op[k];
#pragma unroll
        for (int ch = 0; ch < 2; ++ch) {
            const int child = ch == 0 ? op.c1 : op.c2, m = ch == 0 ? op.m1 : op.m2;
            if (child < 0) {
                if (c == 0) prefetchL1(A.states + (size_t)(-child - 1) * A.Ppad + pp);
                if (m >= 0 && lane < 4) prefetchL1(A.mats + (size_t)m * A.matStride + lane * 4 * CP);
            } else {
                if (!(ch == 0 && (op.flags & 1)) && catValid)
                    prefetchL1(static_cast<const T*>(A.partials) + (size_t)child * A.stride + off0);
                if (m >= 0 && lane == 0) prefetchL1(A.evecs + (size_t)m * CP * 4);
            }
        }
        if (op.sr >= 0 && c == 0) prefetchL1(A.scale + (size_t)op.sr * A.Ppad + pp);
    }
    if (c == 0) {
        prefetchL1(A.patternWeights + pp);
        if (A.cum != nullptr) prefetchL1(A.cum + pp);
    }
    for (int idx = tid; idx < A.nMats * C * 4; idx += 128) {
        const int q = idx / (C * 4), c = (idx >> 2) % C, k = idx & 3;
        sE[q][c][k] = k < S ? exp(A.eval[k] * A.rate[q][c] * A.mat[q].len) : 0.0;
    }
    __syncthreads();
    for (int idx = tid; idx < A.nMats * C * 16; idx += 128) {
        const int q = idx / (C * 16), c = (idx >> 4) % C, j = (idx >> 2) & 3, i = idx & 3;
        double acc = 0.0;
        if (i < S && j < S) {
#pragma unroll
            for (int k = 0; k < 4; ++k) acc += A.V[4 * i + k] * (sE[q][c][k] * A.Vi[4 * k + j]);
            acc = fabs(acc);
        }
        sP[q][c][j * 4 + i] = acc;
        if (blockIdx.x == 0) {
            double* base = A.mats + (size_t)A.mat[q].prob * A.matStride;
            base[((size_t)j * CP + c) * 4 + i] = acc;
            double* mm = base + 16 * CP;
            mm[(size_t)c * 32 + i * 4 + j] = acc;
            mm[(size_t)c * 32 + 16 + i * 4 + j] = 0.0;
            double* mt = mm + (size_t)C * 32;
            mt[(size_t)c * 20 + j * 4 + i] = (j < S) ? acc : ((j == S && i < S) ? 1.0 : 0.0);
            if (j == 0) mt[(size_t)c * 20 + 16 + i] = (S == 4 && i < S) ? 1.0 : 0.0;
            if (j == 0) A.evecs[((size_t)A.mat[q].prob * CP + c) * 4 + i] = sE[q][c][i];
        }
    }
    __syncthreads();

    double d[4] = {0.0, 0.0, 0.0, 0.0};
    for (int k = 0; k < A.nOps; ++k) {
        const IncOp op = A.op[k];
#pragma unroll
        for (int ch = 0; ch < 2; ++ch) {
            const int child = ch == 0 ? op.c1 : op.c2, m = ch == 0 ? op.m1 : op.m2;
            double y[4];
            if (child < 0) {
                const int s = (int)__ldg(A.states + (size_t)(-child - 1) * A.Ppad + pp);
                if (s < S) {
                    if (m < 0) {
                        const double* col = &sP[-m - 1][cc][s * 4];
                        y[0] = col[0]; y[1] = col[1]; y[2] = col[2]; y[3] = col[3];
                    } else {
                        ldg256_ro(A.mats + (size_t)m * A.matStride + ((size_t)s * CP + cc) * 4, y);
                    }
                } else {
#pragma unroll
                    for (int i = 0; i < 4; ++i) y[i] = (i < S) ? 1.0 : 0.0;
                }
            } else {
                double e[4], x[4], u[4];
                if (m < 0) { e[0] = sE[-m - 1][cc][0]; e[1] = sE[-m - 1][cc][1]; e[2] = sE[-m - 1][cc][2]; e[3] = sE[-m - 1][cc][3]; }
                else ldg256_ro(A.evecs + ((size_t)m * CP + cc) * 4, e);
                if (ch == 0 && (op.flags & 1)) {
#pragma unroll
                    for (int i = 0; i < 4; ++i) x[i] = d[i];
                } else {
                    loadCell(static_cast<const T*>(A.partials) + (size_t)child * A.stride + off0, x);
                }
#pragma unroll
                for (int q = 0; q < 4; ++q)
                    u[q] = (A.Vi[4 * q] * x[0] + A.Vi[4 * q + 1] * x[1] + A.Vi[4 * q + 2] * x[2] + A.Vi[4 * q + 3] * x[3]) * e[q];
#pragma unroll
                for (int i = 0; i < 4; ++i)
                    y[i] = absBitsI(A.V[4 * i] * u[0] + A.V[4 * i + 1] * u[1] + A.V[4 * i + 2] * u[2] + A.V[4 * i + 3] * u[3]);
            }
#pragma unroll
            for (int i = 0; i < 4; ++i) d[i] = ch == 0 ? y[i] : d[i] * y[i];
        }
        if (op.sw >= 0) {
            double mx = catValid ? fmax(fmax(d[0], d[1]), fmax(d[2], d[3])) : 0.0;
#pragma unroll
            for (int sh = G; sh < 32; sh <<= 1) mx = fmax(mx, __shfl_xor_sync(0xffffffffu, mx, sh));
            if (mx == 0.0) mx = 1.0;
            const double inv = 1.0 / mx;
#pragma unroll
            for (int i = 0; i < 4; ++i) d[i] *= inv;
            if (c == 0 && inRange) A.scale[(size_t)op.sw * A.Ppad + p] = A.logScalers ? log(mx) : mx;
        } else if (op.sr >= 0) {
            double f = A.scale[(size_t)op.sr * A.Ppad + pp];
            if (A.logScalers) f = exp(f);
            const double inv = 1.0 / f;
#pragma unroll
            for (int i = 0; i < 4; ++i) d[i] *= inv;
        }
        roundCell<T>(d);
        if (catValid && inRange) storeCell(static_cast<T*>(A.partials) + (size_t)op.dest * A.stride + off0, d);
    }

    double t = 0.0;
    if (catValid) t = A.weights[cc] * (A.freqs[0] * d[0] + A.freqs[1] * d[1] + A.freqs[2] * d[2] + A.freqs[3] * d[3]);
#pragma unroll
    for (int sh = G; sh < 32; sh <<= 1) t += __shfl_xor_sync(0xffffffffu, t, sh);
    double contrib = 0.0;
    if (c == 0 && p < A.P) {
        double s = log(t);
        if (A.cum != nullptr) s += A.cum[p];
        A.site[p] = s;
        contrib = A.patternWeights[p] * s;
    }
#pragma unroll
    for (int sh = 16; sh > 0; sh >>= 1) contrib += __shfl_xor_sync(0xffffffffu, contrib, sh);
    if (lane == 0) red[wib] = contrib;
    __syncthreads();
    if (tid == 0) {
        A.blockSums[blockIdx.x] = (red[0] + red[1]) + (red[2] + red[3]);
        __threadfence();
        const unsigned done = atomicAdd(A.counter, 1u);
        last = (done == gridDim.x - 1);
    }
    __syncthreads();
    if (last) {
        __threadfence();
        double acc = 0.0;
        for (int q = tid; q < (int)gridDim.x; q += 128) acc += A.blockSums[q];
#pragma unroll
        for (int sh = 16; sh > 0; sh >>= 1) acc += __shfl_xor_sync(0xffffffffu, acc, sh);
        __syncthreads();
        if (lane == 0) red[wib] = acc;
        __syncthreads();
        if (tid == 0) {
            const double total = (red[0] + red[1]) + (red[2] + red[3]);
            *A.out = total;
            *A.counter = 0u;
            *A.hostOut = total;
            __threadfence_system();
            *A.hostFlag = A.seq;
        }
    }
}

template <int CP>
__global__ void __launch_bounds__(128)
k_incremental(const IncArgs A) {
    incrementalBody<double, CP>(A);
}

template <int CP>
__global__ void __launch_bounds__(128)
k_incrementals(const IncArgs A) {
    incrementalBody<float, CP>(A);
}

}

cudaError_t launchIncremental(Instance* in, const IncArgs& A) {
    const int G = 32 / in->matCP;
    const int blocks = (in->Ppad + 4 * G - 1) / (4 * G);
    if (in->single) {
        switch (in->matCP) {
            case 1: k_incrementals<1><<<blocks, 128, 0, in->stream>>>(A); break;
            case 2: k_incrementals<2><<<blocks, 128, 0, in->stream>>>(A); break;
            case 4: k_incrementals<4><<<blocks, 128, 0, in->stream>>>(A); break;
            case 8: k_incrementals<8><<<blocks, 128, 0, in->stream>>>(A); break;
            default: return cudaErrorInvalidValue;
        }
        return cudaGetLastError();
    }
    switch (in->matCP) {
        case 1: k_incremental<1><<<blocks, 128, 0, in->stream>>>(A); break;
        case 2: k_incremental<2><<<blocks, 128, 0, in->stream>>>(A); break;
        case 4: k_incremental<4><<<blocks, 128, 0, in->stream>>>(A); break;
        case 8: k_incremental<8><<<blocks, 128, 0, in->stream>>>(A); break;
        default: return cudaErrorInvalidValue;
    }
    return cudaGetLastError();
}

}
```

beast-mcmc_b200/csrc/kernels.cu:

```cuda
#include "engine.h"
#include "walk4.cuh"

#include <algorithm>
#include <cfloat>

namespace b200 {

__device__ __forceinline__ void dmma884acc(double& d0, double& d1, double a, double b) {
    asm("mma.sync.aligned.m8n8k4.row.col.f64.f64.f64.f64 {%0,%1}, {%2}, {%3}, {%0,%1};"
        : "+d"(d0), "+d"(d1) : "d"(a), "d"(b));
}

__global__ void k_transition(const double* __restrict__ eigenBase, size_t eigenStride, int S, int Sp, int C,
                             int complexForm, const double* __restrict__ ratesBase,
                             const int* __restrict__ probIdx, const int* __restrict__ eigenIdx,
                             const int* __restrict__ rateSet, const double* __restrict__ lengths,
                             double* __restrict__ matBase, size_t matStride, int matCP, double* __restrict__ evecBase) {
    extern __shared__ double sm[];
    double* ec = sm;
    double* ss = sm + S;
    int* pt = reinterpret_cast<int*>(sm + 2 * S);
    const int b = blockIdx.x, c = blockIdx.y;
    const double* E = eigenBase + (size_t)eigenIdx[b] * eigenStride;
    const double* evec = E;
    const double* ievc = E + (size_t)S * S;
    const double* eval = E + 2 * (size_t)S * S;
    const double d = lengths[b] * ratesBase[(size_t)rateSet[b] * C + c];
    for (int k = threadIdx.x; k < S; k += blockDim.x) {
        double im = complexForm ? eval[S + k] : 0.0;
        if (im == 0.0) {
            ec[k] = exp(d * eval[k]); ss[k] = 0.0; pt[k] = k;
        } else {
            int run = 0;
            for (int q = k - 1; q >= 0 && eval[S + q] != 0.0; --q) ++run;
            const bool first = (run % 2 == 0);
            int k0 = first ? k : k - 1;
            double bb = eval[S + k0];
            double expat = exp(d * eval[k0]);
            ec[k] = expat * cos(d * bb);
            ss[k] = (first ? 1.0 : -1.0) * expat * sin(d * bb);
            pt[k] = first ? k + 1 : k - 1;
        }
    }
    __syncthreads();
    if (evecBase != nullptr && threadIdx.x < 4)
        evecBase[((size_t)probIdx[b] * matCP + c) * 4 + threadIdx.x] = threadIdx.x < S ? ec[threadIdx.x] : 0.0;
    double* out = matBase + (size_t)probIdx[b] * matStride + (matCP ? (size_t)c * 4 : (size_t)c * Sp * Sp);
    const int rowStride = matCP ? matCP * 4 : Sp;
    for (int idx = threadIdx.x; idx < Sp * Sp; idx += blockDim.x) {
        int j = idx / Sp, i = idx % Sp;
        double acc = 0.0;
        if (i < S && j < S) {
            for (int k = 0; k < S; ++k) {
                double iexp = ec[k] * ievc[(size_t)k * S + j] + ss[k] * ievc[(size_t)pt[k] * S + j];
                acc += evec[(size_t)i * S + k] * iexp;
            }
            acc = fabs(acc);
        }
        out[(size_t)j * rowStride + i] = acc;
        if (!matCP) {
            const size_t ld = (size_t)Sp + 4;
            double* padded = matBase + (size_t)probIdx[b] * matStride + (size_t)C * Sp * Sp;
            padded[((size_t)c * Sp + i) * ld + j] = acc;
            padded[(size_t)C * Sp * ld + ((size_t)c * Sp + j) * ld + i] = acc;
        } else {
            double* mm = matBase + (size_t)probIdx[b] * matStride + 16 * matCP;
            mm[(size_t)c * 32 + i * 4 + j] = acc;
            mm[(size_t)c * 32 + 16 + i * 4 + j] = 0.0;
            double* mt = mm + (size_t)C * 32;
            mt[(size_t)c * 20 + j * 4 + i] = (j < S) ? acc : ((j == S && i < S) ? 1.0 : 0.0);
            if (j == 0) mt[(size_t)c * 20 + 16 + i] = (S == 4 && i < S) ? 1.0 : 0.0;
        }
    }
}

__device__ __forceinline__ size_t matEntry(int matCP, int Sp, int c, int i, int j) {
    return matCP ? ((size_t)j * matCP + c) * 4 + i : ((size_t)c * Sp + j) * Sp + i;
}
__global__ void __launch_bounds__(256)
k_combine_matrices(double* __restrict__ matBase, size_t matStride, int S, int Sp, int C, int matCP,
                   const int* __restrict__ first, const int* __restrict__ second, const int* __restrict__ result, int multiply) {
    const int q = blockIdx.x, c = blockIdx.y;
    const double* A = matBase + (size_t)first[q] * matStride;
    const double* B = matBase + (size_t)second[q] * matStride;
    double* R = matBase + (size_t)result[q] * matStride;
    for (int idx = threadIdx.x; idx < Sp * Sp; idx += blockDim.x) {
        const int i = idx / Sp, j = idx % Sp;
        double v = 0.0;
        if (i < S && j < S) {
            if (multiply) for (int k = 0; k < S; ++k) v += A[matEntry(matCP, Sp, c, i, k)] * B[matEntry(matCP, Sp, c, k, j)];
            else v = A[matEntry(matCP, Sp, c, i, j)] + B[matEntry(matCP, Sp, c, i, j)];
        }
        R[matEntry(matCP, Sp, c, i, j)] = v;
        if (!matCP) {
            const size_t ld = (size_t)Sp + 4;
            double* padded = R + (size_t)C * Sp * Sp;
            padded[((size_t)c * Sp + i) * ld + j] = v;
            padded[(size_t)C * Sp * ld + ((size_t)c * Sp + j) * ld + i] = v;
        } else {
            double* mm = R + 16 * matCP;
            mm[(size_t)c * 32 + i * 4 + j] = v;
            mm[(size_t)c * 32 + 16 + i * 4 + j] = 0.0;
            double* mt = mm + (size_t)C * 32;
            mt[(size_t)c * 20 + j * 4 + i] = (j < S) ? v : ((j == S && i < S) ? 1.0 : 0.0);
            if (j == 0) mt[(size_t)c * 20 + 16 + i] = (S == 4 && i < S) ? 1.0 : 0.0;
        }
    }
}

cudaError_t launchCombineMatrices(Instance* in, const int* dFirst, const int* dSecond, const int* dResult, int count, bool multiply) {
    if (count <= 0) return cudaSuccess;
    k_combine_matrices<<<dim3(count, in->C), 256, 0, in->stream>>>(in->dMat, in->matStride, in->S, in->Sp, in->C, in->matCP,
                                                                   dFirst, dSecond, dResult, multiply ? 1 : 0);
    return cudaGetLastError();
}

template <int NT>
__global__ void __launch_bounds__(128)
k_transition_mma(const double* __restrict__ eigenBase, size_t eigenStride, int S, int C,
                 const double* __restrict__ ratesBase, const int* __restrict__ probIdx,
                 const int* __restrict__ eigenIdx, const int* __restrict__ rateSet,
                 const double* __restrict__ lengths, double* __restrict__ matBase, size_t matStride) {
    constexpr int Sp = 8 * NT;
    constexpr int LD = Sp + 4;
    extern __shared__ double smt[];
    double* As = smt;
    double* Bt = smt + Sp * LD;
    double* ex = Bt + Sp * LD;
    const int b = blockIdx.x, c = blockIdx.y, tid = threadIdx.x;
    const double* E = eigenBase + (size_t)eigenIdx[b] * eigenStride;
    const double* evec = E;
    const double* ievc = E + (size_t)S * S;
    const double* eval = E + 2 * (size_t)S * S;
    const double d = lengths[b] * ratesBase[(size_t)rateSet[b] * C + c];
    for (int k = tid; k < Sp; k += 128) ex[k] = k < S ? exp(d * eval[k]) : 0.0;
    __syncthreads();
    for (int q = tid; q < Sp * Sp; q += 128) {
        const int r = q / Sp, col = q % Sp;
        As[r * LD + col] = (r < S && col < S) ? evec[(size_t)r * S + col] : 0.0;
        Bt[col * LD + r] = (r < S && col < S) ? ievc[(size_t)r * S + col] * ex[r] : 0.0;
    }
    __syncthreads();
    const int lane = tid & 31, w = tid >> 5, g = lane >> 2, t = lane & 3;
    double* outT = matBase + (size_t)probIdx[b] * matStride + (size_t)c * Sp * Sp;
    double* outR = matBase + (size_t)probIdx[b] * matStride + (size_t)C * Sp * Sp + (size_t)c * Sp * LD;
    double* outTp = outR + (size_t)C * Sp * LD;
    for (int mt = w; mt < NT; mt += 4) {
        double acc[NT][2];
#pragma unroll
        for (int n = 0; n < NT; ++n) { acc[n][0] = 0.0; acc[n][1] = 0.0; }
        const double* arow = As + (8 * mt + g) * LD + t;
        const double* brow = Bt + g * LD + t;
#pragma unroll 4
        for (int kc = 0; kc < Sp / 4; ++kc) {
            const double a = arow[4 * kc];
#pragma unroll
            for (int n = 0; n < NT; ++n) dmma884acc(acc[n][0], acc[n][1], a, brow[n * 8 * LD + 4 * kc]);
        }
        const int i = 8 * mt + g;
#pragma unroll
        for (int n = 0; n < NT; ++n) {
            const int j = 8 * n + 2 * t;
            const double v0 = fabs(acc[n][0]), v1 = fabs(acc[n][1]);
            *reinterpret_cast<double2*>(outR + (size_t)i * LD + j) = make_double2(v0, v1);
            outT[(size_t)j * Sp + i] = v0;
            outT[(size_t)(j + 1) * Sp + i] = v1;
            outTp[(size_t)j * LD + i] = v0;
            outTp[(size_t)(j + 1) * LD + i] = v1;
        }
    }
}

template <int NT>
static cudaError_t launchTransitionMmaT(Instance* in, const int* dProbIdx, const int* dEigenIdx, const int* dRateSet,
                                        const double* dLengths, int count) {
    constexpr int Sp = 8 * NT;
    const size_t smem = (2 * (size_t)Sp * (Sp + 4) + Sp) * sizeof(double);
    static_assert(Sp <= 64, "shared-memory budget");
    cudaError_t e = cudaFuncSetAttribute(k_transition_mma<NT>, cudaFuncAttributeMaxDynamicSharedMemorySize, (int)smem);
    if (e != cudaSuccess) return e;
    dim3 grid(count, in->C);
    k_transition_mma<NT><<<grid, 128, smem, in->stream>>>(in->dEigen, 2 * (size_t)in->S * in->S + 2 * in->S, in->S, in->C,
                                                          in->dRates, dProbIdx, dEigenIdx, dRateSet, dLengths, in->dMat,
                                                          in->matStride);
    return cudaGetLastError();
}

cudaError_t launchTransitionMatrices(Instance* in, const int* dProbIdx, const int* dEigenIdx,
                                     const int* dRateSet, const double* dLengths, int count) {
    if (count <= 0) return cudaSuccess;
    if (in->genericMma && in->matCP == 0 && !in->complexEigen) {
        switch (in->Sp / 8) {
            case 1: return launchTransitionMmaT<1>(in, dProbIdx, dEigenIdx, dRateSet, dLengths, count);
            case 2: return launchTransitionMmaT<2>(in, dProbIdx, dEigenIdx, dRateSet, dLengths, count);
            case 3: return launchTransitionMmaT<3>(in, dProbIdx, dEigenIdx, dRateSet, dLengths, count);
            case 4: return launchTransitionMmaT<4>(in, dProbIdx, dEigenIdx, dRateSet, dLengths, count);
            case 8: return launchTransitionMmaT<8>(in, dProbIdx, dEigenIdx, dRateSet, dLengths, count);
            default: break;
        }
    }
    size_t smem = (size_t)in->S * (2 * sizeof(double) + sizeof(int)) + 16;
    int threads = in->Sp * in->Sp >= 1024 ? 256 : (in->Sp * in->Sp >= 128 ? 128 : 32);
    dim3 grid(count, in->C);
    k_transition<<<grid, threads, smem, in->stream>>>(in->dEigen, 2 * (size_t)in->S * in->S + 2 * in->S, in->S,
                                                      in->Sp, in->C, in->complexEigen ? 1 : 0, in->dRates,
                                                      dProbIdx, dEigenIdx, dRateSet, dLengths, in->dMat,
                                                      in->matStride, in->matCP, in->matCP ? in->dEvec : nullptr);
    return cudaGetLastError();
}

struct Mat4 { double r[4][4]; };

template <int CP>
__device__ __forceinline__ void loadMat(const double* __restrict__ m, Mat4& M) {
    ldg256_ro(m, M.r[0]); ldg256_ro(m + 4 * CP, M.r[1]); ldg256_ro(m + 8 * CP, M.r[2]); ldg256_ro(m + 12 * CP, M.r[3]);
}

__device__ __forceinline__ void applyMat(const Mat4& M, const double (&x)[4], double (&y)[4]) {
#pragma unroll
    for (int i = 0; i < 4; ++i) y[i] = M.r[0][i] * x[0] + M.r[1][i] * x[1] + M.r[2][i] * x[2] + M.r[3][i] * x[3];
}

template <typename T, int CP, int R, bool STACK, bool FIRST>
__device__ __forceinline__ void childTerm(const WalkArgs& A, int child, int matIdx, int slot, int moff, size_t off0,
                                          int p0, bool catValid, int pBegin, int pEnd, const double2* stackMem,
                                          int nthreads, double (&y)[R][4]) {
    constexpr int G = 32 / CP;
    const int S = A.S;
    const double* m = A.mats + (size_t)matIdx * A.matStride + moff;
    if (child < 0) {
        const uint8_t* t = A.states + (size_t)(-child - 1) * A.Ppad;
#pragma unroll
        for (int r = 0; r < R; ++r) {
            const int p = p0 + r * G;
            const bool active = catValid && p >= pBegin && p < pEnd;
            const int s = active ? (int)__ldg(t + p) : S;
            double v[4];
            if (s < S) ldg256_ro(m + 4 * CP * s, v);
            else {
#pragma unroll
                for (int i = 0; i < 4; ++i) v[i] = (i < S) ? 1.0 : 0.0;
            }
#pragma unroll
            for (int i = 0; i < 4; ++i) y[r][i] = FIRST ? v[i] : y[r][i] * v[i];
        }
    } else {
        Mat4 M;
        loadMat<CP>(m, M);
        const T* xg = static_cast<const T*>(A.partials) + (size_t)child * A.stride + off0;
#pragma unroll
        for (int r = 0; r < R; ++r) {
            const int p = p0 + r * G;
            const bool active = catValid && p >= pBegin && p < pEnd;
            double x[4], v[4];
            if (STACK && slot != 0xFF) {
                double2 lo = stackMem[((slot * R + r) * 2 + 0) * nthreads + threadIdx.x];
                double2 hi = stackMem[((slot * R + r) * 2 + 1) * nthreads + threadIdx.x];
                x[0] = lo.x; x[1] = lo.y; x[2] = hi.x; x[3] = hi.y;
            } else if (active) {
                loadCell(xg + (size_t)r * G * 4, x);
            } else { x[0] = x[1] = x[2] = x[3] = 0.0; }
            applyMat(M, x, v);
#pragma unroll
            for (int i = 0; i < 4; ++i) y[r][i] = FIRST ? v[i] : y[r][i] * v[i];
        }
    }
}

template <typename T, int CP, int R, bool STACK, bool PRE>
__device__ __forceinline__ void walk4Body(const WalkArgs& A) {
    static_assert(sizeof(T) == 8 || !STACK, "the operand-stack variant is built for fp64 partials only");
    constexpr int G = 32 / CP;
    extern __shared__ double2 stackMem[];
    const int lane = threadIdx.x & 31;
    const int warp = (blockIdx.x * blockDim.x + threadIdx.x) >> 5;
    const int c = lane / G;
    const int4 range = __ldg(A.subs + blockIdx.y);
    const int p0 = range.z + warp * (G * R) + (lane % G);
    if (range.z + warp * (G * R) >= range.w) return;
    const bool catValid = c < A.C;
    const int cc = catValid ? c : 0;
    const size_t off0 = ((size_t)cc * A.Ppad + p0) * 4;
    const int moff = cc * 4;
    const int nthreads = blockDim.x;
    const int last = range.y - 1;

    Op4 cur = loadOp(A.ops + range.x);
    double d[R][4];
#pragma unroll
    for (int r = 0; r < R; ++r) d[r][0] = d[r][1] = d[r][2] = d[r][3] = 0.0;
    for (int k = range.x; k <= last; ++k) {
        Op4 nxt;
        if (R == 1) nxt = loadOp(A.ops + min(k + 1, last));
        else if (lane == 0) prefetchL1(A.ops + min(k + 2, last));
        const int s1 = cur.slots & 0xFF, s2 = (cur.slots >> 8) & 0xFF, sd = (cur.slots >> 16) & 0xFF;
        if (!STACK) {
#pragma unroll
            for (int w = 0; w < 2; ++w) {
                const int pf = w == 0 ? cur.pfA : cur.pfB;
                if (pf == 0) continue;
                if (pf & 1) {
                    const uint8_t* t = A.states + (size_t)(pf >> 1) * A.Ppad + p0;
                    if ((lane % G) == 0 && c == 0) prefetchL1(t);
                } else if (catValid) {
                    const T* xg = static_cast<const T*>(A.partials) + (size_t)((pf >> 1) - 1) * A.stride + off0;
#pragma unroll
                    for (int r = 0; r < R; ++r)
                        if (p0 + r * G < A.Ppad) prefetchL1(xg + (size_t)r * G * 4);
                }
            }
            if (lane < 8) {
                const int mi = lane < 4 ? cur.pfM1 : cur.pfM2;
                if (mi >= 0) prefetchL1(A.mats + (size_t)mi * A.matStride + (lane & 3) * 4 * CP);
            }
        }
        if (!PRE) {
            if (!STACK && (cur.pad_ & 2)) {
                Mat4 M;
                loadMat<CP>(A.mats + (size_t)cur.m1 * A.matStride + moff, M);
#pragma unroll
                for (int r = 0; r < R; ++r) {
                    double v[4];
                    applyMat(M, d[r], v);
#pragma unroll
                    for (int i = 0; i < 4; ++i) d[r][i] = v[i];
                }
            } else {
                childTerm<T, CP, R, STACK, true>(A, cur.c1, cur.m1, s1, moff, off0, p0, catValid, cur.pBegin, cur.pEnd, stackMem, nthreads, d);
            }
            childTerm<T, CP, R, STACK, false>(A, cur.c2, cur.m2, s2, moff, off0, p0, catValid, cur.pBegin, cur.pEnd, stackMem, nthreads, d);
        } else {
            double v[R][4];
            childTerm<T, CP, R, false, true>(A, cur.c2, cur.m2, 0xFF, moff, off0, p0, catValid, cur.pBegin, cur.pEnd, stackMem, nthreads, v);
            Mat4 M1;
            loadMat<CP>(A.mats + (size_t)cur.m1 * A.matStride + moff, M1);
            const T* xg = static_cast<const T*>(A.partials) + (size_t)cur.c1 * A.stride + off0;
            const bool fromRegisters = (cur.pad_ & 2) != 0;
#pragma unroll
            for (int r = 0; r < R; ++r) {
                const int p = p0 + r * G;
                double x[4] = {0.0, 0.0, 0.0, 0.0};
                if (fromRegisters) {
#pragma unroll
                    for (int i = 0; i < 4; ++i) x[i] = d[r][i];
                } else if (catValid && p >= cur.pBegin && p < cur.pEnd) loadCell(xg + (size_t)r * G * 4, x);
                double q[4];
#pragma unroll
                for (int i = 0; i < 4; ++i) q[i] = x[i] * v[r][i];
#pragma unroll
                for (int j = 0; j < 4; ++j) d[r][j] = M1.r[j][0] * q[0] + M1.r[j][1] * q[1] + M1.r[j][2] * q[2] + M1.r[j][3] * q[3];
            }
        }
        if (R != 1) nxt = loadOp(A.ops + min(k + 1, last));
        T* dg = static_cast<T*>(A.partials) + (size_t)cur.dest * A.stride + off0;
#pragma unroll
        for (int r = 0; r < R; ++r) {
            const int p = p0 + r * G;
            const bool active = catValid && p >= cur.pBegin && p < cur.pEnd;
            if (cur.sw >= 0) {
                double m = active ? fmax(fmax(d[r][0], d[r][1]), fmax(d[r][2], d[r][3])) : 0.0;
#pragma unroll
                for (int sh = G; sh < 32; sh <<= 1) m = fmax(m, __shfl_xor_sync(0xffffffffu, m, sh));
                if (m == 0.0) m = 1.0;
                const double inv = 1.0 / m;
#pragma unroll
                for (int i = 0; i < 4; ++i) d[r][i] *= inv;
                if (active && c == 0) {
                    A.scale[(size_t)cur.sw * A.Ppad + p] = A.logScalers ? log(m) : m;
                }
                __syncwarp();
            } else if (cur.sr >= 0) {
                double f = active ? A.scale[(size_t)cur.sr * A.Ppad + p] : 1.0;
                if (A.logScalers) f = exp(f);
                const double inv = 1.0 / f;
// ... 1633 lines not shown
```

beast-mcmc_b200/csrc/walk4.cuh:

```cuda
#pragma once
#include "engine.h"

namespace b200 {

__device__ __forceinline__ void ldg256(const double* p, double (&v)[4]) {
    asm volatile("ld.global.v2.f64 {%0,%1}, [%4];\n\tld.global.v2.f64 {%2,%3}, [%4+16];"
                 : "=d"(v[0]), "=d"(v[1]), "=d"(v[2]), "=d"(v[3]) : "l"(p) : "memory");
}
__device__ __forceinline__ void ldg256_nc(const double* p, double (&v)[4]) {
    asm volatile("ld.global.nc.v2.f64 {%0,%1}, [%4];\n\tld.global.nc.v2.f64 {%2,%3}, [%4+16];"
                 : "=d"(v[0]), "=d"(v[1]), "=d"(v[2]), "=d"(v[3]) : "l"(p));
}
__device__ __forceinline__ void stg256(double* p, const double (&v)[4]) {
    asm volatile("st.global.v2.f64 [%0], {%1,%2};\n\tst.global.v2.f64 [%0+16], {%3,%4};"
                 :: "l"(p), "d"(v[0]), "d"(v[1]), "d"(v[2]), "d"(v[3]) : "memory");
}

template <typename T>
__device__ __forceinline__ void roundCell(double (&v)[4]) {
    if constexpr (sizeof(T) == 4) {
#pragma unroll
        for (int i = 0; i < 4; ++i) {
            float f;
            asm("cvt.rn.f32.f64 %0, %1;" : "=f"(f) : "d"(v[i]));
            const unsigned b = __float_as_uint(f);
            v[i] = (double)((b & 0x7f800000u) ? f : __uint_as_float(b & 0x80000000u));
        }
    }
}
__device__ __forceinline__ void loadCell(const double* p, double (&v)[4]) { ldg256(p, v); }
__device__ __forceinline__ void loadCell(const float* p, double (&v)[4]) {
    float f[4];
    asm volatile("ld.global.v4.f32 {%0,%1,%2,%3}, [%4];" : "=f"(f[0]), "=f"(f[1]), "=f"(f[2]), "=f"(f[3]) : "l"(p) : "memory");
#pragma unroll
    for (int i = 0; i < 4; ++i) v[i] = f[i];
}
__device__ __forceinline__ void storeCell(double* p, const double (&v)[4]) { stg256(p, v); }
__device__ __forceinline__ void storeCell(float* p, const double (&v)[4]) {
    asm volatile("st.global.v4.f32 [%0], {%1,%2,%3,%4};"
                 :: "l"(p), "f"((float)v[0]), "f"((float)v[1]), "f"((float)v[2]), "f"((float)v[3]) : "memory");
}

struct WalkArgs {
    const Op4* ops;
    const int4* subs;
    void* partials;
    size_t stride;
    const uint8_t* states;
    const double* mats;
    double* scale;
    int S, C, Ppad, logScalers;
    size_t matStride;
    int matMmaOffset;
    const double* evecs;
    const double* recipes;
    const int4* virtTips;
    double V[16];
    double Vi[16];
};

__device__ __forceinline__ Op4 loadOp(const Op4* p) {
    const int4* q = reinterpret_cast<const int4*>(p);
    int4 a = __ldg(q), b = __ldg(q + 1), c = __ldg(q + 2), d = __ldg(q + 3);
    Op4 o;
    o.dest = a.x; o.c1 = a.y; o.c2 = a.z; o.m1 = a.w;
    o.m2 = b.x; o.sw = b.y; o.sr = b.z; o.cum = b.w;
    o.pBegin = c.x; o.pEnd = c.y; o.slots = (unsigned)c.z; o.pad_ = c.w;
    o.pfA = d.x; o.pfB = d.y; o.pfM1 = d.z; o.pfM2 = d.w;
    return o;
}

__device__ __forceinline__ void prefetchL1(const void* p) {
    asm volatile("prefetch.global.L1 [%0];" :: "l"(p));
}

__device__ __forceinline__ void ldg256_ro(const double* p, double (&v)[4]) {
    asm("ld.global.nc.v2.f64 {%0,%1}, [%4];\n\tld.global.nc.v2.f64 {%2,%3}, [%4+16];"
        : "=d"(v[0]), "=d"(v[1]), "=d"(v[2]), "=d"(v[3]) : "l"(p));
}
__device__ __forceinline__ void loadCellRo(const double* p, double (&v)[4]) { ldg256_ro(p, v); }
__device__ __forceinline__ void loadCellRo(const float* p, double (&v)[4]) {
    float f[4];
    asm("ld.global.nc.v4.f32 {%0,%1,%2,%3}, [%4];" : "=f"(f[0]), "=f"(f[1]), "=f"(f[2]), "=f"(f[3]) : "l"(p));
#pragma unroll
    for (int i = 0; i < 4; ++i) v[i] = f[i];
}

}
```

beast-mcmc_b200/csrc/walk4e.cu:

```cuda
#include "engine.h"
#include "walk4.cuh"

namespace b200 {

namespace {

__device__ __forceinline__ double absBits(double v) {
    return __hiloint2double(__double2hiint(v) & 0x7fffffff, __double2loint(v));
}

template <typename T, int CP, int R, bool ALIGNED, bool FIRST, int TIP>
__device__ __forceinline__ void childTermE(const WalkArgs& A, const double (&Vi)[16], int child, int matIdx, bool fromRegisters,
                                           int cc, size_t off0, int p0, bool catValid, int pBegin, int pEnd, double (&d)[R][4],
                                           double* tab) {
    constexpr int G = 32 / CP;
    const int S = A.S;
    const bool tip = child < 0;
    if (TIP == 2 && tip) {
        const int lane = threadIdx.x & 31;
        const uint8_t* t = A.states + (size_t)(-child - 1) * A.Ppad;
        int s[R];
#pragma unroll
        for (int r = 0; r < R; ++r) {
            const int p = p0 + r * G;
            s[r] = (ALIGNED || (catValid && p >= pBegin && p < pEnd)) ? (int)__ldg(t + p) : 4;
        }
        const double* m = A.mats + (size_t)matIdx * A.matStride;
        __syncwarp();
#pragma unroll
        for (int q = lane; q < 5 * CP; q += 32) {
            const int c = q / 5, sym = q - 5 * c;
            double v[4];
            if (sym < S && sym < 4 && c < A.C) ldg256_ro(m + (sym * CP + c) * 4, v);
            else {
#pragma unroll
                for (int i = 0; i < 4; ++i) v[i] = (i < S) ? 1.0 : 0.0;
            }
            double2* dst = reinterpret_cast<double2*>(tab + q * 4);
            dst[0] = make_double2(v[0], v[1]);
            dst[1] = make_double2(v[2], v[3]);
        }
        __syncwarp();
#pragma unroll
        for (int r = 0; r < R; ++r) {
            const double2* col = reinterpret_cast<const double2*>(tab + (cc * 5 + min(s[r], 4)) * 4);
            const double2 lo = col[0], hi = col[1];
            if (FIRST) { d[r][0] = lo.x; d[r][1] = lo.y; d[r][2] = hi.x; d[r][3] = hi.y; }
            else { d[r][0] *= lo.x; d[r][1] *= lo.y; d[r][2] *= hi.x; d[r][3] *= hi.y; }
        }
        return;
    }
    if (TIP == 1 && tip) {
        const uint8_t* t = A.states + (size_t)(-child - 1) * A.Ppad;
        const double* m = A.mats + (size_t)matIdx * A.matStride + cc * 4;
#pragma unroll
        for (int r = 0; r < R; ++r) {
            const int p = p0 + r * G;
            const int s = (ALIGNED || (catValid && p >= pBegin && p < pEnd)) ? (int)__ldg(t + p) : S;
            double v[4];
            if (s < S) ldg256_ro(m + 4 * CP * s, v);
            else {
#pragma unroll
                for (int i = 0; i < 4; ++i) v[i] = (i < S) ? 1.0 : 0.0;
            }
#pragma unroll
            for (int i = 0; i < 4; ++i) d[r][i] = FIRST ? v[i] : d[r][i] * v[i];
        }
        return;
    }
    double e[4];
    ldg256_ro(A.evecs + ((size_t)matIdx * CP + cc) * 4, e);
    const uint8_t* t = A.states + (size_t)(tip ? -child - 1 : 0) * A.Ppad;
    const T* xg = static_cast<const T*>(A.partials) + (size_t)(tip ? 0 : child) * A.stride + off0;
#pragma unroll
    for (int r = 0; r < R; ++r) {
        const int p = p0 + r * G;
        const bool live = ALIGNED || (catValid && p >= pBegin && p < pEnd);
        double x[4], u[4], y[4];
        int s = 0;
        if (tip) {
            s = live ? (int)__ldg(t + p) : S;
#pragma unroll
            for (int j = 0; j < 4; ++j) x[j] = (s == j) ? 1.0 : 0.0;
        } else if (fromRegisters) {
#pragma unroll
            for (int i = 0; i < 4; ++i) x[i] = d[r][i];
        } else if (live) {
            loadCell(xg + (size_t)r * G * 4, x);
        } else {
            x[0] = x[1] = x[2] = x[3] = 0.0;
        }
#pragma unroll
        for (int k = 0; k < 4; ++k)
            u[k] = (Vi[4 * k] * x[0] + Vi[4 * k + 1] * x[1] + Vi[4 * k + 2] * x[2] + Vi[4 * k + 3] * x[3]) * e[k];
#pragma unroll
        for (int i = 0; i < 4; ++i)
            y[i] = absBits(A.V[4 * i] * u[0] + A.V[4 * i + 1] * u[1] + A.V[4 * i + 2] * u[2] + A.V[4 * i + 3] * u[3]);
        if (tip && s >= S) {
#pragma unroll
            for (int i = 0; i < 4; ++i) y[i] = (i < S) ? 1.0 : 0.0;
        }
#pragma unroll
        for (int i = 0; i < 4; ++i) d[r][i] = FIRST ? y[i] : d[r][i] * y[i];
    }
}

template <typename T, int CP, int R, bool ALIGNED, int TIP>
__device__ __forceinline__ void walk4eBody(const WalkArgs& A) {
    constexpr int G = 32 / CP;
    const int lane = threadIdx.x & 31;
    const int warp = (blockIdx.x * blockDim.x + threadIdx.x) >> 5;
    const int c = lane / G;
    const int4 range = __ldg(A.subs + blockIdx.y);
    const int p0 = range.z + warp * (G * R) + (lane % G);
    if (range.z + warp * (G * R) >= range.w) return;
    const bool catValid = c < A.C;
    const int cc = catValid ? c : 0;
    const size_t off0 = ((size_t)cc * A.Ppad + p0) * 4;
    const int last = range.y - 1;
    __shared__ __align__(16) double tipTab[TIP == 2 ? 4 * 2 * CP * 20 : 2];
    double* tab1 = tipTab + (TIP == 2 ? ((threadIdx.x >> 5) * 2) * CP * 20 : 0);
    double* tab2 = tab1 + (TIP == 2 ? CP * 20 : 0);

    double Vi[16];
#pragma unroll
    for (int q = 0; q < 16; ++q) asm volatile("mov.f64 %0, %1;" : "=d"(Vi[q]) : "d"(A.Vi[q]));
    Op4 cur = loadOp(A.ops + range.x);
    double d[R][4];
#pragma unroll
    for (int r = 0; r < R; ++r) d[r][0] = d[r][1] = d[r][2] = d[r][3] = 0.0;
    for (int k = range.x; k <= last; ++k) {
        Op4 nxt;
        if (R == 1) nxt = loadOp(A.ops + min(k + 1, last));
        else if (lane == 0) prefetchL1(A.ops + min(k + 2, last));
#pragma unroll
        for (int w = 0; w < 2; ++w) {
            const int pf = w == 0 ? cur.pfA : cur.pfB;
            if (pf == 0) continue;
            if (pf & 1) {
                const uint8_t* t = A.states + (size_t)(pf >> 1) * A.Ppad + p0;
                if ((lane % G) == 0 && c == 0) prefetchL1(t);
            } else if (catValid) {
                const T* xg = static_cast<const T*>(A.partials) + (size_t)((pf >> 1) - 1) * A.stride + off0;
#pragma unroll
                for (int r = 0; r < R; ++r)
                    if (ALIGNED || p0 + r * G < A.Ppad) prefetchL1(xg + (size_t)r * G * 4);
            }
        }
        if (lane < 2) {
            const int mi = lane == 0 ? cur.pfM1 : cur.pfM2;
            if (mi >= 0) prefetchL1(A.evecs + (size_t)mi * CP * 4);
        } else if (TIP != 0 && lane >= 8 && lane < 16) {
            const int mi = lane < 12 ? cur.pfM1 : cur.pfM2;
            if (mi >= 0) prefetchL1(A.mats + (size_t)mi * A.matStride + (lane & 3) * 4 * CP);
        }
        childTermE<T, CP, R, ALIGNED, true, TIP>(A, Vi, cur.c1, cur.m1, (cur.pad_ & 2) != 0, cc, off0, p0, catValid, cur.pBegin, cur.pEnd, d, tab1);
        childTermE<T, CP, R, ALIGNED, false, TIP>(A, Vi, cur.c2, cur.m2, false, cc, off0, p0, catValid, cur.pBegin, cur.pEnd, d, tab2);
        if (R != 1) nxt = loadOp(A.ops + min(k + 1, last));
        T* dg = static_cast<T*>(A.partials) + (size_t)cur.dest * A.stride + off0;
#pragma unroll
        for (int r = 0; r < R; ++r) {
            const int p = p0 + r * G;
            const bool active = ALIGNED ? catValid : (catValid && p >= cur.pBegin && p < cur.pEnd);
            if (cur.sw >= 0) {
                double m = active ? fmax(fmax(d[r][0], d[r][1]), fmax(d[r][2], d[r][3])) : 0.0;
#pragma unroll
                for (int sh = G; sh < 32; sh <<= 1) m = fmax(m, __shfl_xor_sync(0xffffffffu, m, sh));
                if (m == 0.0) m = 1.0;
                const double inv = 1.0 / m;
#pragma unroll
                for (int i = 0; i < 4; ++i) d[r][i] *= inv;
                if (active && c == 0) A.scale[(size_t)cur.sw * A.Ppad + p] = A.logScalers ? log(m) : m;
            } else if (cur.sr >= 0) {
                double f = active ? A.scale[(size_t)cur.sr * A.Ppad + p] : 1.0;
                if (A.logScalers) f = exp(f);
                const double inv = 1.0 / f;
#pragma unroll
                for (int i = 0; i < 4; ++i) d[r][i] *= inv;
            }
            roundCell<T>(d[r]);
            if (active) storeCell(dg + (size_t)r * G * 4, d[r]);
        }
        cur = nxt;
    }
}

template <int CP, int R, bool ALIGNED, int MINB, int TIP>
__global__ void __launch_bounds__(128, MINB)
k_walk4e(const WalkArgs A) {
    walk4eBody<double, CP, R, ALIGNED, TIP>(A);
}

template <int CP, int R, bool ALIGNED, int MINB, int TIP>
__global__ void __launch_bounds__(128, MINB)
k_walk4es(const WalkArgs A) {
    walk4eBody<float, CP, R, ALIGNED, TIP>(A);
}

__device__ __forceinline__ void cpAsync16(void* smemDst, const void* gmemSrc) {
    const unsigned sAddr = (unsigned)__cvta_generic_to_shared(smemDst);
    asm volatile("cp.async.ca.shared.global [%0], [%1], 16;" :: "r"(sAddr), "l"(gmemSrc) : "memory");
}
template <int BYTES>
__device__ __forceinline__ void cpAsyncSmall(void* smemDst, const void* gmemSrc) {
    const unsigned sAddr = (unsigned)__cvta_generic_to_shared(smemDst);
    asm volatile("cp.async.ca.shared.global [%0], [%1], %2;" :: "r"(sAddr), "l"(gmemSrc), "n"(BYTES) : "memory");
}

template <int CP, int R, bool VIRT>
struct WarpStage {
    static constexpr int G = 32 / CP, NP = G * R, TABLES = VIRT ? 4 : 2;
    double mat[TABLES][5 * CP * 4];
    double ev[2][CP * 4];
    alignas(16) unsigned char st[TABLES][NP < 16 ? 16 : NP];
};

template <typename T, int CP, int R, bool VIRT>
__device__ __forceinline__ void walk4pBody(const WalkArgs& A) {
    constexpr int G = 32 / CP, NP = G * R;
    constexpr int PIECE = NP < 16 ? NP : 16;
    static_assert(NP % PIECE == 0 && (PIECE == 4 || PIECE == 8 || PIECE == 16), "state-byte staging");
    constexpr int TABLES = WarpStage<CP, R, VIRT>::TABLES;
    constexpr int RECQ = sizeof(Op4) / 16 + (VIRT ? 1 : 0);
    __shared__ __align__(16) WarpStage<CP, R, VIRT> stages[4][2];
    __shared__ __align__(16) Op4 rings[4][4];
    __shared__ __align__(16) int4 tipRings[4][VIRT ? 4 : 1];
    int lane;
    asm volatile("mov.u32 %0, %%laneid;" : "=r"(lane));
    const int wib = threadIdx.x >> 5;
    const int warp = (blockIdx.x * blockDim.x + threadIdx.x) >> 5;
    const int c = lane / G;
    const int4 range = __ldg(A.subs + blockIdx.y);
    const int pBase = range.z + warp * NP;
    if (pBase >= range.w) return;
    const int p0 = pBase + (lane % G);
    const bool catValid = c < A.C;
    const int cc = catValid ? c : 0;
    const size_t off0 = ((size_t)cc * A.Ppad + p0) * 4;
    const int last = range.y - 1, S = A.S;
    WarpStage<CP, R, VIRT>* stage = stages[wib];
    Op4* ring = rings[wib];
    int4* tipRing = tipRings[wib];

    for (int q = lane; q < 2 * TABLES * CP * 4; q += 32) {
        const int tbl = q / (CP * 4), e = q % (CP * 4), gc = e >> 2, i = e & 3;
        stage[tbl / TABLES].mat[tbl % TABLES][(i >> 1) * 10 * CP + 2 * (4 * CP + gc) + (i & 1)] = (i < S) ? 1.0 : 0.0;
    }
    auto stageBlock = [&](double* tab, const double* src) {
#pragma unroll
        for (int q = lane; q < CP * 8; q += 32)
            cpAsync16(&tab[(q & 1) * 10 * CP + 2 * (((q >> 1) % CP) * 4 + q / (2 * CP))], src + 2 * q);
    };
    auto fetchRecord = [&](int j) {
        if (VIRT && lane == RECQ - 1) cpAsync16(&tipRing[j & 3], A.virtTips + j);
        else cpAsync16(reinterpret_cast<char*>(&ring[j & 3]) + 16 * lane, reinterpret_cast<const char*>(A.ops + j) + 16 * lane);
    };
    struct Rec { int dest, c1, c2, sw, sr, flags, pfA, pfB; };
    auto issueOperands = [&](int j) -> Rec {
        const int4 rec = *reinterpret_cast<const int4*>(&ring[j & 3]);
        const int4 rec2 = *(reinterpret_cast<const int4*>(&ring[j & 3]) + 1);
        const int flags = ring[j & 3].pad_;
        const int2 pf = *reinterpret_cast<const int2*>(&ring[j & 3].pfA);
        const int m2 = rec2.x;
        WarpStage<CP, R, VIRT>& sg = stage[j & 1];
#pragma unroll
        for (int ch = 0; ch < 2; ++ch) {
            const int child = ch == 0 ? rec.y : rec.z, m = ch == 0 ? rec.w : m2;
            const bool virt = VIRT && (flags & (4 << ch)) != 0;
            if (child < 0) {
                stageBlock(sg.mat[ch], A.mats + (size_t)m * A.matStride);
            } else {
                if (virt) {
                    const double* rcp = A.recipes + (size_t)child * 32 * CP;
                    stageBlock(sg.mat[ch], rcp);
                    stageBlock(sg.mat[TABLES - 2 + ch], rcp + 16 * CP);
                }
                if (lane < CP * 2) cpAsync16(&sg.ev[ch][2 * lane], A.evecs + (size_t)m * CP * 4 + 2 * lane);
            }
        }
        constexpr int SL = NP / PIECE;
        auto statePiece = [&](int q) {
            const int t = q / SL, piece = q % SL, ch = t & 1;
            const int child = ch == 0 ? rec.y : rec.z;
            int tip = t < 2 && child < 0 ? -child - 1 : -1;
            if (VIRT && (flags & (4 << ch)) != 0) {
                const int4 vt = tipRing[j & 3];
                tip = t == 0 ? vt.x : t == 1 ? vt.z : t == 2 ? vt.y : vt.w;
            }
            if (tip >= 0) cpAsyncSmall<PIECE>(&sg.st[t][PIECE * piece], A.states + (size_t)tip * A.Ppad + pBase + PIECE * piece);
        };
        if (lane < RECQ) {
            if (j + 1 <= last) fetchRecord(j + 1);
        } else if (lane < RECQ + TABLES * SL) {
            statePiece(lane - RECQ);
        }
        if constexpr (RECQ + TABLES * SL > 32) {
            if (lane < RECQ + TABLES * SL - 32) statePiece(lane + 32 - RECQ);
        }
        asm volatile("cp.async.commit_group;" ::: "memory");
        return Rec{rec.x, rec.y, rec.z, rec2.y, rec2.z, flags, pf.x, pf.y};
    };
    if (lane < RECQ) fetchRecord(range.x);
    asm volatile("cp.async.commit_group;" ::: "memory");
    asm volatile("cp.async.wait_group 0;" ::: "memory");
    __syncwarp();
    Rec nxt = issueOperands(range.x);
    asm volatile("cp.async.wait_group 0;" ::: "memory");
    __syncwarp();

    double Vi[16];
#pragma unroll
    for (int q = 0; q < 16; ++q) asm volatile("mov.f64 %0, %1;" : "=d"(Vi[q]) : "d"(A.Vi[q]));
    double d[R][4];
#pragma unroll
    for (int r = 0; r < R; ++r) d[r][0] = d[r][1] = d[r][2] = d[r][3] = 0.0;

    for (int k = range.x; k <= last; ++k) {
        const Rec cur = nxt;
        if (k + 1 <= last) nxt = issueOperands(k + 1);
        const WarpStage<CP, R, VIRT>& sg = stage[k & 1];
#pragma unroll
        for (int w = 0; w < 2; ++w) {
            const int pf = w == 0 ? cur.pfA : cur.pfB;
            if (pf == 0 || (pf & 1) || !catValid) continue;
            const T* xg = static_cast<const T*>(A.partials) + (size_t)((pf >> 1) - 1) * A.stride + off0;
#pragma unroll
            for (int r = 0; r < R; ++r) prefetchL1(xg + (size_t)r * G * 4);
        }
#pragma unroll
        for (int ch = 0; ch < 2; ++ch) {
            const int child = ch == 0 ? cur.c1 : cur.c2;
            if (child < 0) {
#pragma unroll
                for (int r = 0; r < R; ++r) {
                    const int sym = sg.st[ch][(lane % G) + r * G];
                    const int e2 = 2 * (sym < S ? cc * 4 + sym : 4 * CP + cc);
                    const double2 lo = *reinterpret_cast<const double2*>(&sg.mat[ch][e2]);
                    const double2 hi = *reinterpret_cast<const double2*>(&sg.mat[ch][10 * CP + e2]);
                    if (ch == 0) { d[r][0] = lo.x; d[r][1] = lo.y; d[r][2] = hi.x; d[r][3] = hi.y; }
                    else { d[r][0] *= lo.x; d[r][1] *= lo.y; d[r][2] *= hi.x; d[r][3] *= hi.y; }
                }
            } else {
                const double2* ep = reinterpret_cast<const double2*>(&sg.ev[ch][cc * 4]);
                const double2 e01 = ep[0], e23 = ep[1];
                const double e[4] = {e01.x, e01.y, e23.x, e23.y};
                const bool fromRegisters = ch == 0 && (cur.flags & 2) != 0;
                const bool virt = VIRT && (cur.flags & (4 << ch)) != 0;
                const T* xg = static_cast<const T*>(A.partials) + (size_t)child * A.stride + off0;
#pragma unroll
                for (int r = 0; r < R; ++r) {
                    double x[4], u[4], y[4];
                    if (fromRegisters) {
#pragma unroll
                        for (int i = 0; i < 4; ++i) x[i] = d[r][i];
                    } else if (virt) {
                        const int symA = sg.st[ch][(lane % G) + r * G], symB = sg.st[TABLES - 2 + ch][(lane % G) + r * G];
                        const int eA = 2 * (symA < S ? cc * 4 + symA : 4 * CP + cc);
                        const int eB = 2 * (symB < S ? cc * 4 + symB : 4 * CP + cc);
                        const double2 aLo = *reinterpret_cast<const double2*>(&sg.mat[ch][eA]);
                        const double2 aHi = *reinterpret_cast<const double2*>(&sg.mat[ch][10 * CP + eA]);
                        const double2 bLo = *reinterpret_cast<const double2*>(&sg.mat[TABLES - 2 + ch][eB]);
                        const double2 bHi = *reinterpret_cast<const double2*>(&sg.mat[TABLES - 2 + ch][10 * CP + eB]);
                        x[0] = aLo.x * bLo.x; x[1] = aLo.y * bLo.y; x[2] = aHi.x * bHi.x; x[3] = aHi.y * bHi.y;
                        roundCell<T>(x);
                    } else {
                        loadCell(xg + (size_t)r * G * 4, x);
                    }
#pragma unroll
                    for (int q = 0; q < 4; ++q)
                        u[q] = (Vi[4 * q] * x[0] + Vi[4 * q + 1] * x[1] + Vi[4 * q + 2] * x[2] + Vi[4 * q + 3] * x[3]) * e[q];
#pragma unroll
                    for (int i = 0; i < 4; ++i)
                        y[i] = absBits(A.V[4 * i] * u[0] + A.V[4 * i + 1] * u[1] + A.V[4 * i + 2] * u[2] + A.V[4 * i + 3] * u[3]);
#pragma unroll
                    for (int i = 0; i < 4; ++i) d[r][i] = ch == 0 ? y[i] : d[r][i] * y[i];
                }
            }
        }
        T* dg = static_cast<T*>(A.partials) + (size_t)cur.dest * A.stride + off0;
#pragma unroll
        for (int r = 0; r < R; ++r) {
            const int p = p0 + r * G;
            if (cur.sw >= 0) {
                double m = catValid ? fmax(fmax(d[r][0], d[r][1]), fmax(d[r][2], d[r][3])) : 0.0;
#pragma unroll
                for (int sh = G; sh < 32; sh <<= 1) m = fmax(m, __shfl_xor_sync(0xffffffffu, m, sh));
                if (m == 0.0) m = 1.0;
                const double inv = 1.0 / m;
#pragma unroll
                for (int i = 0; i < 4; ++i) d[r][i] *= inv;
                if (c == 0) A.scale[(size_t)cur.sw * A.Ppad + p] = A.logScalers ? log(m) : m;
            } else if (cur.sr >= 0) {
                double f = A.scale[(size_t)cur.sr * A.Ppad + p];
                if (A.logScalers) f = exp(f);
                const double inv = 1.0 / f;
#pragma unroll
                for (int i = 0; i < 4; ++i) d[r][i] *= inv;
            }
            roundCell<T>(d[r]);
            if (catValid) storeCell(dg + (size_t)r * G * 4, d[r]);
        }
        asm volatile("cp.async.wait_group 0;" ::: "memory");
        __syncwarp();
    }
}

template <int CP, int R, int MINB>
__global__ void __launch_bounds__(128, MINB)
k_walk4p(const WalkArgs A) {
    walk4pBody<double, CP, R, false>(A);
}

template <int CP, int R, int MINB>
__global__ void __launch_bounds__(128, MINB)
k_walk4ps(const WalkArgs A) {
    walk4pBody<float, CP, R, false>(A);
}

template <int CP, int R, int MINB>
__global__ void __launch_bounds__(128, MINB)
k_walk4pv(const WalkArgs A) {
    walk4pBody<double, CP, R, true>(A);
}

template <int CP, int R, int MINB>
__global__ void __launch_bounds__(128, MINB)
k_walk4pvs(const WalkArgs A) {
    walk4pBody<float, CP, R, true>(A);
}

template <typename T, int CP, int R, int MINB>
cudaError_t launchP(Instance* in, const WalkArgs& A, dim3 grid) {
    if constexpr (sizeof(T) == 4) k_walk4ps<CP, R, MINB><<<grid, 128, 0, in->stream>>>(A);
    else k_walk4p<CP, R, MINB><<<grid, 128, 0, in->stream>>>(A);
    return cudaGetLastError();
}

template <typename T, int CP, int R>
cudaError_t launchPV(Instance* in, const WalkArgs& A, dim3 grid) {
    if constexpr (sizeof(T) == 4) k_walk4pvs<CP, R, 3><<<grid, 128, 0, in->stream>>>(A);
    else k_walk4pv<CP, R, 3><<<grid, 128, 0, in->stream>>>(A);
    return cudaGetLastError();
}

__global__ void k_cherry_snapshot(const int4* items, const double* mats, size_t matStride, double* recipes, int blk) {
    const int4 it = items[blockIdx.x];
    for (int q = threadIdx.x; q < 2 * blk; q += blockDim.x)
        recipes[(size_t)it.x * 2 * blk + q] = mats[(size_t)(q < blk ? it.y : it.z) * matStride + q % blk];
}

template <typename T>
__device__ __forceinline__ void cherryStoreBody(const int4* items, int count, T* partials, size_t stride,
                                                const uint8_t* states, const double* recipes, int S, int C, int CP, int Ppad) {
    const int q = blockIdx.x * blockDim.x + threadIdx.x;
    if (q >= C * Ppad) return;
    const int c = q / Ppad, p = q - c * Ppad;
    for (int k = blockIdx.y; k < count; k += gridDim.y) {
        const int4 it = items[k];
        const int sA = states[(size_t)it.z * Ppad + p], sB = states[(size_t)it.w * Ppad + p];
        const double* ra = recipes + (size_t)it.y * 32 * CP;
        const double* rb = ra + 16 * CP;
        double v[4];
#pragma unroll
        for (int i = 0; i < 4; ++i) {
            const double a = sA < S ? ra[(sA * CP + c) * 4 + i] : (i < S ? 1.0 : 0.0);
            const double b = sB < S ? rb[(sB * CP + c) * 4 + i] : (i < S ? 1.0 : 0.0);
            v[i] = a * b;
        }
        roundCell<T>(v);
        storeCell(partials + (size_t)it.x * stride + (size_t)q * 4, v);
    }
}

__global__ void k_cherry_store(const int4* items, int count, double* partials, size_t stride, const uint8_t* states,
                               const double* recipes, int S, int C, int CP, int Ppad) {
    cherryStoreBody(items, count, partials, stride, states, recipes, S, C, CP, Ppad);
}

__global__ void k_cherry_store_f32(const int4* items, int count, float* partials, size_t stride, const uint8_t* states,
                                const double* recipes, int S, int C, int CP, int Ppad) {
    cherryStoreBody(items, count, partials, stride, states, recipes, S, C, CP, Ppad);
}

template <typename T, int CP, int R, bool ALIGNED, int MINB, int TIP>
cudaError_t launchK(Instance* in, const WalkArgs& A, dim3 grid) {
    if constexpr (sizeof(T) == 4) k_walk4es<CP, R, ALIGNED, MINB, TIP><<<grid, 128, 0, in->stream>>>(A);
    else k_walk4e<CP, R, ALIGNED, MINB, TIP><<<grid, 128, 0, in->stream>>>(A);
    return cudaGetLastError();
}

int phaseR(const Instance* in, int nSubs, int maxWindow) {
    const int G = 32 / in->matCP;
    const long walks = (long)nSubs * ((maxWindow + G * in->walkR - 1) / (G * in->walkR));
    if ((in->thinR1 && walks < (long)in->smCount * 8) || in->walkR == 1) return 1;
    if (in->matCP == 4 && (in->walkR == 8 || in->walkR == 2)) return in->walkR;
    return 4;
}

bool stagedWalk(const Instance* in, int R, bool aligned) {
    const int G = 32 / in->matCP;
    return aligned && in->Ppad % (G * R) == 0 && in->matCP <= 8 && G * R >= 4 && (R == 1 ? in->thinTipMode : in->tipMode) == 3;
}

template <typename T, int CP, int R>
cudaError_t launchR(Instance* in, WalkArgs& A, int nSubs, int maxWindow, bool aligned, bool virt) {
    constexpr int G = 32 / CP;
    constexpr int TIPD = CP <= 8 ? 2 : 0;
    const int warps = (maxWindow + G * R - 1) / (G * R);
    dim3 grid((warps + 3) / 4, nSubs);
    if constexpr (CP <= 8 && G * R >= 4) {
        if (stagedWalk(in, R, aligned)) {
            if (virt) {
                if constexpr (R == 8) return cudaErrorInvalidValue;
                else return launchPV<T, CP, R>(in, A, grid);
            }
            if constexpr (CP == 4) {
                const int minb = in->walkMinBlocksSet ? in->walkMinBlocks : 3;
                if (minb >= 6) return launchP<T, CP, R, 6>(in, A, grid);
                if (minb == 5) return launchP<T, CP, R, 5>(in, A, grid);
                if (minb == 3) return launchP<T, CP, R, 3>(in, A, grid);
            }
            return launchP<T, CP, R, 4>(in, A, grid);
        }
    }
    if (virt) return cudaErrorInvalidValue;
    if (!aligned || in->Ppad % (G * R) != 0) return launchK<T, CP, R, false, 4, TIPD>(in, A, grid);
    if constexpr (CP == 4 && R >= 2) {
        const int minb = in->walkMinBlocks, tip = in->tipMode;
        if (tip == 0) {
            if (minb >= 5) return launchK<T, CP, R, true, 5, 0>(in, A, grid);
            if (minb == 3) return launchK<T, CP, R, true, 3, 0>(in, A, grid);
            return launchK<T, CP, R, true, 4, 0>(in, A, grid);
        }
        if (tip == 1) {
            if (minb >= 5) return launchK<T, CP, R, true, 5, 1>(in, A, grid);
            return launchK<T, CP, R, true, 4, 1>(in, A, grid);
        }
        if (minb >= 6) return launchK<T, CP, R, true, 6, 2>(in, A, grid);
        if (minb == 5) return launchK<T, CP, R, true, 5, 2>(in, A, grid);
        if (minb == 3) return launchK<T, CP, R, true, 3, 2>(in, A, grid);
    }
    return launchK<T, CP, R, true, 4, TIPD>(in, A, grid);
}

template <typename T, int CP>
cudaError_t launchCP(Instance* in, WalkArgs& A, int nSubs, int maxWindow, bool aligned, bool virt) {
    const int R = phaseR(in, nSubs, maxWindow);
    if (R == 1) return launchR<T, CP, 1>(in, A, nSubs, maxWindow, aligned, virt);
    if constexpr (CP == 4) {
        if (R == 8) return launchR<T, CP, 8>(in, A, nSubs, maxWindow, aligned, virt);
        if (R == 2) return launchR<T, CP, 2>(in, A, nSubs, maxWindow, aligned, virt);
    }
    return launchR<T, CP, 4>(in, A, nSubs, maxWindow, aligned, virt);
}

}

bool walk4pServes(const Instance* in, int nSubs, int maxWindow) {
    if (in->matCP == 0) return false;
    const int R = phaseR(in, nSubs, maxWindow);
    return R != 8 && stagedWalk(in, R, true);
}

cudaError_t launchWalk4E(Instance* in, const Op4* dOps, const int4* dSubs, int nSubs, int maxWindow, bool aligned,
                         const double* eigen, const int4* dVirtTips) {
    const bool virt = dVirtTips != nullptr;
    if (nSubs <= 0) return cudaSuccess;
    WalkArgs A;
    A.ops = dOps; A.subs = dSubs; A.partials = in->partialsBase; A.stride = in->partialsElems;
    A.states = in->states8Base; A.mats = in->dMat; A.scale = in->dScale;
    A.S = in->S; A.C = in->C; A.Ppad = in->Ppad; A.logScalers = in->logScalers ? 1 : 0;
    A.matStride = in->matStride; A.matMmaOffset = 16 * in->matCP;
    A.evecs = in->dEvec;
    A.recipes = in->dRecipe;
    A.virtTips = dVirtTips;
    if (virt && in->dRecipe == nullptr) return cudaErrorInvalidValue;
    for (int q = 0; q < 16; ++q) { A.V[q] = eigen[q]; A.Vi[q] = eigen[16 + q]; }
    if (in->single) {
        switch (in->matCP) {
            case 1: return launchCP<float, 1>(in, A, nSubs, maxWindow, aligned, virt);
            case 2: return launchCP<float, 2>(in, A, nSubs, maxWindow, aligned, virt);
            case 8: return launchCP<float, 8>(in, A, nSubs, maxWindow, aligned, virt);
            default: return launchCP<float, 4>(in, A, nSubs, maxWindow, aligned, virt);
        }
    }
    switch (in->matCP) {
#ifndef B200_W4E_QUICK
        case 1: return launchCP<double, 1>(in, A, nSubs, maxWindow, aligned, virt);
        case 2: return launchCP<double, 2>(in, A, nSubs, maxWindow, aligned, virt);
        case 8: return launchCP<double, 8>(in, A, nSubs, maxWindow, aligned, virt);
        case 16: return launchCP<double, 16>(in, A, nSubs, maxWindow, aligned, virt);
        case 32: return launchCP<double, 32>(in, A, nSubs, maxWindow, aligned, virt);
#endif
        default: return launchCP<double, 4>(in, A, nSubs, maxWindow, aligned, virt);
    }
}

cudaError_t launchCherrySnapshot(Instance* in, const int4* dItems, int count) {
    if (count <= 0) return cudaSuccess;
    k_cherry_snapshot<<<count, 128, 0, in->stream>>>(dItems, in->dMat, in->matStride, in->dRecipe, 16 * in->matCP);
    return cudaGetLastError();
}

cudaError_t launchCherryStore(Instance* in, const int4* dItems, int count) {
    if (count <= 0) return cudaSuccess;
    const dim3 grid((in->C * in->Ppad + 255) / 256, std::min(count, 65535));
    if (in->single)
        k_cherry_store_f32<<<grid, 256, 0, in->stream>>>(dItems, count, reinterpret_cast<float*>(in->partialsBase),
                                                      in->partialsElems, in->states8Base, in->dRecipe, in->S, in->C,
                                                      in->matCP, in->Ppad);
    else
        k_cherry_store<<<grid, 256, 0, in->stream>>>(dItems, count, reinterpret_cast<double*>(in->partialsBase),
                                                     in->partialsElems, in->states8Base, in->dRecipe, in->S, in->C,
                                                     in->matCP, in->Ppad);
    return cudaGetLastError();
}

cudaError_t updateWalk4EGraph(cudaGraphExec_t exec, const std::vector<cudaGraphNode_t>& kernelNodes, const double* eigen) {
    for (cudaGraphNode_t node : kernelNodes) {
        cudaKernelNodeParams kp;
        cudaError_t e = cudaGraphKernelNodeGetParams(node, &kp);
        if (e != cudaSuccess) return e;
        if (kp.func == reinterpret_cast<void*>(k_cherry_snapshot)) continue;
        if (kp.kernelParams == nullptr || kp.kernelParams[0] == nullptr) return cudaErrorInvalidValue;
        WalkArgs A = *static_cast<const WalkArgs*>(kp.kernelParams[0]);
        for (int q = 0; q < 16; ++q) { A.V[q] = eigen[q]; A.Vi[q] = eigen[16 + q]; }
        void* args[1] = {&A};
        kp.kernelParams = args;
        kp.extra = nullptr;
        e = cudaGraphExecKernelNodeSetParams(exec, node, &kp);
        if (e != cudaSuccess) return e;
    }
    return cudaSuccess;
}

}
```

Before: 2249.

## Replace eigen-form child transform with staged full transition matrices

The walk kernels used to push each child partial through V·diag(e)·Vi, using per-matrix eigenvalue exponentials plus V/Vi passed as kernel arguments. They now stage the precomputed 4x4 transition matrix into shared memory and apply it directly. This removes the evec buffer, the per-call eigen kernel arguments and the graph-node parameter patching, so cached graphs no longer need updating when the eigen system changes. In exchange, shared-memory staging per warp grows, moving to dynamic shared memory with an opt-in above 48KB for CP=8, and more matrix bytes are loaded per child.

```diff
diff --git a/beast-mcmc_b200/csrc/api.cu b/beast-mcmc_b200/csrc/api.cu
--- a/beast-mcmc_b200/csrc/api.cu
+++ b/beast-mcmc_b200/csrc/api.cu
@@ -141,7 +141,7 @@
     if (in->stream) cudaStreamSynchronize(in->stream);
     cudaFree(in->partialsBase); cudaFree(in->states8Base); cudaFree(in->states32Base);
     for (CachedPlan& cp : in->planCache) { cp.dropGraph(); cudaFree(cp.dBlock); }
-    cudaFree(in->dEigen); cudaFree(in->dMat); cudaFree(in->dEvec); cudaFree(in->dIncSums); cudaFree(in->dIncCounter);
+    cudaFree(in->dEigen); cudaFree(in->dMat); cudaFree(in->dIncSums); cudaFree(in->dIncCounter);
     cudaFree(in->dRecipe);
     if (in->hMapped) cudaFreeHost(in->hMapped); cudaFree(in->dRates); cudaFree(in->dWeights);
     cudaFree(in->dFreqs); cudaFree(in->dScale); cudaFree(in->dPatternWeights);
@@ -397,7 +397,7 @@
         TimedScope ts(in, T_PARTIALS);
         if (fourPath && eigenSlot >= 0 && !preOrder && (ph >= phaseDepth.size() || phaseDepth[ph] == 0)) {
             e = launchWalk4E(in, static_cast<const Op4*>(dOps), static_cast<const int4*>(dSubs) + s0, s1 - s0, maxWindow,
-                             aligned, in->hEigen.data() + (size_t)eigenSlot * 36, static_cast<const int4*>(dVirtTips));
+                             aligned, static_cast<const int4*>(dVirtTips));
             continue;
         }
         if (virt) return cudaErrorInvalidValue;
@@ -526,20 +526,14 @@
             CUDA_OK(storeExternal(in, cp.external));
             cp.lastUse = ++in->planClock;
             cp.hits++;
-            const unsigned eigenGenNow = eigenSlot >= 0 ? in->eigenGen[eigenSlot] : 0u;
+            const int eigenForm = eigenSlot >= 0 ? 1 : 0;
             const void* dSnap = static_cast<char*>(cp.dBlock) + cp.snapOffset;
             const int nSnap = (int)cp.cherries.size();
             const void* dTips = cp.readsVirtual ? static_cast<char*>(cp.dBlock) + cp.tipsOffset : nullptr;
-            if (cp.graphExec != nullptr && (cp.graphEigen != eigenSlot || cp.graphEigenGen != eigenGenNow)) {
-                if (cp.graphAllEigen && eigenSlot >= 0 && cp.graphEigen == eigenSlot &&
-                    updateWalk4EGraph(cp.graphExec, cp.graphKernelNodes, in->hEigen.data() + (size_t)eigenSlot * 36) == cudaSuccess) {
-                    cp.graphEigenGen = eigenGenNow;
-                } else {
-                    cudaGetLastError();
-                    cp.dropGraph();
-                    cp.hits = 1;
-                    if (++cp.graphInvalidations >= 4) cp.graphFailed = true;
-                }
+            if (cp.graphExec != nullptr && cp.graphEigenForm != eigenForm) {
+                cp.dropGraph();
+                cp.hits = 1;
+                if (++cp.graphInvalidations >= 4) cp.graphFailed = true;
             }
             int launches = nSnap > 0;
             for (size_t ph = 0; ph + 1 < cp.phaseStart.size(); ++ph) launches += cp.phaseStart[ph + 1] > cp.phaseStart[ph];
@@ -549,31 +543,15 @@
                     const cudaError_t e1 = launchPlan(in, cp.dBlock, static_cast<char*>(cp.dBlock) + cp.subsOffset, cp.phaseStart,
                                                       cp.phaseDepth, cp.fourPath, cp.maxWindow, cp.preOrder, eigenSlot,
                                                       !cp.byPartition, dSnap, nSnap, dTips);
-                    cp.graphEigen = eigenSlot;
-                    cp.graphEigenGen = eigenGenNow;
+                    cp.graphEigenForm = eigenForm;
                     cudaGraph_t g = nullptr;
                     const cudaError_t e2 = cudaStreamEndCapture(in->stream, &g);
                     if (e1 != cudaSuccess || e2 != cudaSuccess || g == nullptr ||
                         cudaGraphInstantiate(&cp.graphExec, g, 0) != cudaSuccess) {
                         cp.graphExec = nullptr;
                         cp.graphFailed = true;
-                        if (g) cudaGraphDestroy(g);
-                    } else {
-                        cp.graph = g;
-                        cp.graphKernelNodes.clear();
-                        cp.graphAllEigen = cp.fourPath && eigenSlot >= 0 && !cp.preOrder;
-                        for (int dpt : cp.phaseDepth) cp.graphAllEigen = cp.graphAllEigen && dpt == 0;
-                        size_t nn = 0;
-                        if (cudaGraphGetNodes(g, nullptr, &nn) == cudaSuccess && nn > 0) {
-                            std::vector<cudaGraphNode_t> nodes(nn);
-                            cudaGraphNodeType ty;
-                            if (cudaGraphGetNodes(g, nodes.data(), &nn) == cudaSuccess)
-                                for (size_t q = 0; q < nn; ++q)
-                                    if (cudaGraphNodeGetType(nodes[q], &ty) == cudaSuccess && ty == cudaGraphNodeTypeKernel)
-                                        cp.graphKernelNodes.push_back(nodes[q]);
-                        }
-                        if (cp.graphKernelNodes.empty()) cp.graphAllEigen = false;
                     }
+                    if (g) cudaGraphDestroy(g);
                     if (getenv("B200_BEAGLE_DEBUG"))
                         fprintf(stderr, "[b200-beagle] graph %s: %d launches\n", cp.graphExec ? "captured" : "capture failed",
                                 launches);
@@ -1088,6 +1066,7 @@
     in->tipMode = envInt("B200_TIP_MODE", 3);
     in->thinTipMode = envInt("B200_THIN_TIP_MODE", in->tipMode);
     in->virtualCherries = envInt("B200_VIRTUAL_CHERRIES", 1);
+    in->debug = getenv("B200_BEAGLE_DEBUG") != nullptr;
     in->walkBlock = 128;
     in->walkVariant = envInt("B200_WALK_VARIANT", 0);
     in->reorder = envInt("B200_REORDER", 1);
@@ -1135,12 +1114,12 @@
     };
     alloc(&in->dEigen, std::max(1, in->nEigen) * eigenStride);
     alloc(&in->dMat, matElems);
-    if (in->matCP > 0) alloc(&in->dEvec, (size_t)in->nMatrices * in->matCP * 4);
     if (in->matCP > 0 && in->matCP <= 8 && in->virtualCherries) {
         alloc(&in->dRecipe, (size_t)in->nBuffers * 32 * in->matCP);
         in->cherryTip1.assign(in->nBuffers, -1);
         in->cherryTip2.assign(in->nBuffers, -1);
         in->cherryStored.assign(in->nBuffers, 0);
+        ok = ok && configureWalk4E(in) == cudaSuccess;
     }
     if (in->matCP > 0 && in->matCP <= 8) {
         alloc(&in->dIncSums, (size_t)in->Ppad / 4 + 8);
@@ -1525,7 +1504,7 @@
     IncArgs A;
     memset(&A, 0, sizeof A);
     A.partials = in->partialsBase; A.stride = in->partialsElems; A.states = in->states8Base; A.mats = in->dMat;
-    A.evecs = in->dEvec; A.scale = in->dScale; A.matStride = in->matStride;
+    A.scale = in->dScale; A.matStride = in->matStride;
     A.S = in->S; A.C = in->C; A.Ppad = in->Ppad; A.P = in->P; A.logScalers = in->logScalers ? 1 : 0;
     const double* h = in->hEigen.data() + (size_t)E * 36;
     for (int q = 0; q < 16; ++q) { A.V[q] = h[q]; A.Vi[q] = h[16 + q]; }
diff --git a/beast-mcmc_b200/csrc/engine.h b/beast-mcmc_b200/csrc/engine.h
--- a/beast-mcmc_b200/csrc/engine.h
+++ b/beast-mcmc_b200/csrc/engine.h
@@ -55,16 +55,11 @@
     long hits = 0;
     cudaGraphExec_t graphExec = nullptr;
     bool graphFailed = false;
-    int graphEigen = -2;
-    unsigned graphEigenGen = 0;
+    int graphEigenForm = -1;
     int graphInvalidations = 0;
-    cudaGraph_t graph = nullptr;
-    std::vector<cudaGraphNode_t> graphKernelNodes;
-    bool graphAllEigen = false;
     void dropGraph() {
         if (graphExec) cudaGraphExecDestroy(graphExec);
-        if (graph) cudaGraphDestroy(graph);
-        graphExec = nullptr; graph = nullptr; graphKernelNodes.clear(); graphAllEigen = false;
+        graphExec = nullptr;
     }
 };
 
@@ -74,7 +69,7 @@
 struct IncOp { int dest, c1, c2, m1, m2, sw, sr, flags; };
 struct IncMat { int prob, rateSet; double len; };
 struct IncArgs {
-    void* partials; size_t stride; const uint8_t* states; double* mats; double* evecs; double* scale;
+    void* partials; size_t stride; const uint8_t* states; double* mats; double* scale;
     size_t matStride;
     int S, C, Ppad, P, logScalers, nOps, nMats, pad_;
     double V[16], Vi[16], eval[4];
@@ -121,7 +116,6 @@
 
     double* dEigen = nullptr;
     double* dMat = nullptr;
-    double* dEvec = nullptr;
     std::vector<int> matEigen;
     std::vector<unsigned> matEigenGen, eigenGen;
     std::vector<char> eigenReal;
@@ -148,6 +142,7 @@
     int lookaheadPre = 1;
     int prePhases = 1;
     int useGraphs = 1;
+    bool debug = false;
     int lookahead = 1;
     int forward = 1;
     double* dScratch = nullptr;
@@ -216,10 +211,10 @@
 cudaError_t launchTransitionMatrices(Instance* in, const int* dProbIdx, const int* dEigenIdx,
                                      const int* dRateSet, const double* dLengths, int count);
 cudaError_t launchWalk4(Instance* in, const Op4* dOps, const int4* dSubs, int nSubs, int stackDepth, int maxWindow, bool preOrder);
-cudaError_t updateWalk4EGraph(cudaGraphExec_t exec, const std::vector<cudaGraphNode_t>& kernelNodes, const double* eigen);
 cudaError_t launchWalk4E(Instance* in, const Op4* dOps, const int4* dSubs, int nSubs, int maxWindow, bool aligned,
-                         const double* eigen, const int4* dVirtTips);
+                         const int4* dVirtTips);
 bool walk4pServes(const Instance* in, int nSubs, int maxWindow);
+cudaError_t configureWalk4E(const Instance* in);
 cudaError_t launchCherrySnapshot(Instance* in, const int4* dItems, int count);
 cudaError_t launchCherryStore(Instance* in, const int4* dItems, int count);
 cudaError_t launchWalkGeneric(Instance* in, const DevOp* dOps, const int4* dSubs, int nSubs, int maxWindow, bool preOrder);
diff --git a/beast-mcmc_b200/csrc/incr.cu b/beast-mcmc_b200/csrc/incr.cu
--- a/beast-mcmc_b200/csrc/incr.cu
+++ b/beast-mcmc_b200/csrc/incr.cu
@@ -4,10 +4,6 @@
 namespace b200 {
 
 namespace {
-
-__device__ __forceinline__ double absBitsI(double v) {
-    return __hiloint2double(__double2hiint(v) & 0x7fffffff, __double2loint(v));
-}
 
 template <typename T, int CP>
 __device__ __forceinline__ void incrementalBody(const IncArgs& A) {
@@ -36,7 +32,7 @@
             } else {
                 if (!(ch == 0 && (op.flags & 1)) && catValid)
                     prefetchL1(static_cast<const T*>(A.partials) + (size_t)child * A.stride + off0);
-                if (m >= 0 && lane == 0) prefetchL1(A.evecs + (size_t)m * CP * 4);
+                if (m >= 0 && lane < 4) prefetchL1(A.mats + (size_t)m * A.matStride + lane * 4 * CP);
             }
         }
         if (op.sr >= 0 && c == 0) prefetchL1(A.scale + (size_t)op.sr * A.Ppad + pp);
@@ -47,7 +43,7 @@
     }
     for (int idx = tid; idx < A.nMats * C * 4; idx += 128) {
         const int q = idx / (C * 4), c = (idx >> 2) % C, k = idx & 3;
-        sE[q][c][k] = k < S ? exp(A.eval[k] * A.rate[q][c] * A.mat[q].len) : 0.0;
+        sE[q][c][k] = k < S ? exp((A.mat[q].len * A.rate[q][c]) * A.eval[k]) : 0.0;
     }
     __syncthreads();
     for (int idx = tid; idx < A.nMats * C * 16; idx += 128) {
@@ -68,7 +64,6 @@
             double* mt = mm + (size_t)C * 32;
             mt[(size_t)c * 20 + j * 4 + i] = (j < S) ? acc : ((j == S && i < S) ? 1.0 : 0.0);
             if (j == 0) mt[(size_t)c * 20 + 16 + i] = (S == 4 && i < S) ? 1.0 : 0.0;
-            if (j == 0) A.evecs[((size_t)A.mat[q].prob * CP + c) * 4 + i] = sE[q][c][i];
         }
     }
     __syncthreads();
@@ -94,21 +89,26 @@
                     for (int i = 0; i < 4; ++i) y[i] = (i < S) ? 1.0 : 0.0;
                 }
             } else {
-                double e[4], x[4], u[4];
-                if (m < 0) { e[0] = sE[-m - 1][cc][0]; e[1] = sE[-m - 1][cc][1]; e[2] = sE[-m - 1][cc][2]; e[3] = sE[-m - 1][cc][3]; }
-                else ldg256_ro(A.evecs + ((size_t)m * CP + cc) * 4, e);
+                Mat4 M;
+                double x[4];
+                if (m < 0) {
+                    const double* pc = sP[-m - 1][cc];
+#pragma unroll
+                    for (int j = 0; j < 4; ++j) {
+                        const double2 lo = *reinterpret_cast<const double2*>(pc + 4 * j);
+                        const double2 hi = *reinterpret_cast<const double2*>(pc + 4 * j + 2);
+                        M.r[j][0] = lo.x; M.r[j][1] = lo.y; M.r[j][2] = hi.x; M.r[j][3] = hi.y;
+                    }
+                } else {
+                    loadMat<CP>(A.mats + (size_t)m * A.matStride + cc * 4, M);
+                }
                 if (ch == 0 && (op.flags & 1)) {
 #pragma unroll
                     for (int i = 0; i < 4; ++i) x[i] = d[i];
                 } else {
                     loadCell(static_cast<const T*>(A.partials) + (size_t)child * A.stride + off0, x);
                 }
-#pragma unroll
-                for (int q = 0; q < 4; ++q)
-                    u[q] = (A.Vi[4 * q] * x[0] + A.Vi[4 * q + 1] * x[1] + A.Vi[4 * q + 2] * x[2] + A.Vi[4 * q + 3] * x[3]) * e[q];
-#pragma unroll
-                for (int i = 0; i < 4; ++i)
-                    y[i] = absBitsI(A.V[4 * i] * u[0] + A.V[4 * i + 1] * u[1] + A.V[4 * i + 2] * u[2] + A.V[4 * i + 3] * u[3]);
+                applyMat(M, x, y);
             }
 #pragma unroll
             for (int i = 0; i < 4; ++i) d[i] = ch == 0 ? y[i] : d[i] * y[i];
diff --git a/beast-mcmc_b200/csrc/kernels.cu b/beast-mcmc_b200/csrc/kernels.cu
--- a/beast-mcmc_b200/csrc/kernels.cu
+++ b/beast-mcmc_b200/csrc/kernels.cu
@@ -15,7 +15,7 @@
                              int complexForm, const double* __restrict__ ratesBase,
                              const int* __restrict__ probIdx, const int* __restrict__ eigenIdx,
                              const int* __restrict__ rateSet, const double* __restrict__ lengths,
-                             double* __restrict__ matBase, size_t matStride, int matCP, double* __restrict__ evecBase) {
+                             double* __restrict__ matBase, size_t matStride, int matCP) {
     extern __shared__ double sm[];
     double* ec = sm;
     double* ss = sm + S;
@@ -43,8 +43,6 @@
         }
     }
     __syncthreads();
-    if (evecBase != nullptr && threadIdx.x < 4)
-        evecBase[((size_t)probIdx[b] * matCP + c) * 4 + threadIdx.x] = threadIdx.x < S ? ec[threadIdx.x] : 0.0;
     double* out = matBase + (size_t)probIdx[b] * matStride + (matCP ? (size_t)c * 4 : (size_t)c * Sp * Sp);
     const int rowStride = matCP ? matCP * 4 : Sp;
     for (int idx = threadIdx.x; idx < Sp * Sp; idx += blockDim.x) {
@@ -205,21 +203,10 @@
     k_transition<<<grid, threads, smem, in->stream>>>(in->dEigen, 2 * (size_t)in->S * in->S + 2 * in->S, in->S,
                                                       in->Sp, in->C, in->complexEigen ? 1 : 0, in->dRates,
                                                       dProbIdx, dEigenIdx, dRateSet, dLengths, in->dMat,
-                                                      in->matStride, in->matCP, in->matCP ? in->dEvec : nullptr);
+                                                      in->matStride, in->matCP);
     return cudaGetLastError();
 }
 
-struct Mat4 { double r[4][4]; };
-
-template <int CP>
-__device__ __forceinline__ void loadMat(const double* __restrict__ m, Mat4& M) {
-    ldg256_ro(m, M.r[0]); ldg256_ro(m + 4 * CP, M.r[1]); ldg256_ro(m + 8 * CP, M.r[2]); ldg256_ro(m + 12 * CP, M.r[3]);
-}
-
-__device__ __forceinline__ void applyMat(const Mat4& M, const double (&x)[4], double (&y)[4]) {
-#pragma unroll
-    for (int i = 0; i < 4; ++i) y[i] = M.r[0][i] * x[0] + M.r[1][i] * x[1] + M.r[2][i] * x[2] + M.r[3][i] * x[3];
-}
 
 template <typename T, int CP, int R, bool STACK, bool FIRST>
 __device__ __forceinline__ void childTerm(const WalkArgs& A, int child, int matIdx, int slot, int moff, size_t off0,
diff --git a/beast-mcmc_b200/csrc/walk4.cuh b/beast-mcmc_b200/csrc/walk4.cuh
--- a/beast-mcmc_b200/csrc/walk4.cuh
+++ b/beast-mcmc_b200/csrc/walk4.cuh
@@ -52,11 +52,8 @@
     int S, C, Ppad, logScalers;
     size_t matStride;
     int matMmaOffset;
-    const double* evecs;
     const double* recipes;
     const int4* virtTips;
-    double V[16];
-    double Vi[16];
 };
 
 __device__ __forceinline__ Op4 loadOp(const Op4* p) {
@@ -86,4 +83,16 @@
     for (int i = 0; i < 4; ++i) v[i] = f[i];
 }
 
+struct Mat4 { double r[4][4]; };
+
+template <int CP>
+__device__ __forceinline__ void loadMat(const double* __restrict__ m, Mat4& M) {
+    ldg256_ro(m, M.r[0]); ldg256_ro(m + 4 * CP, M.r[1]); ldg256_ro(m + 8 * CP, M.r[2]); ldg256_ro(m + 12 * CP, M.r[3]);
 }
+
+__device__ __forceinline__ void applyMat(const Mat4& M, const double (&x)[4], double (&y)[4]) {
+#pragma unroll
+    for (int i = 0; i < 4; ++i) y[i] = M.r[0][i] * x[0] + M.r[1][i] * x[1] + M.r[2][i] * x[2] + M.r[3][i] * x[3];
+}
+
+}
diff --git a/beast-mcmc_b200/csrc/walk4e.cu b/beast-mcmc_b200/csrc/walk4e.cu
--- a/beast-mcmc_b200/csrc/walk4e.cu
+++ b/beast-mcmc_b200/csrc/walk4e.cu
@@ -1,16 +1,14 @@
 #include "engine.h"
 #include "walk4.cuh"
 
+#include <cstdio>
+
 namespace b200 {
 
 namespace {
 
-__device__ __forceinline__ double absBits(double v) {
-    return __hiloint2double(__double2hiint(v) & 0x7fffffff, __double2loint(v));
-}
-
 template <typename T, int CP, int R, bool ALIGNED, bool FIRST, int TIP>
-__device__ __forceinline__ void childTermE(const WalkArgs& A, const double (&Vi)[16], int child, int matIdx, bool fromRegisters,
+__device__ __forceinline__ void childTermE(const WalkArgs& A, int child, int matIdx, bool fromRegisters,
                                            int cc, size_t off0, int p0, bool catValid, int pBegin, int pEnd, double (&d)[R][4],
                                            double* tab) {
     constexpr int G = 32 / CP;
@@ -68,15 +66,15 @@
         }
         return;
     }
-    double e[4];
-    ldg256_ro(A.evecs + ((size_t)matIdx * CP + cc) * 4, e);
+    Mat4 M;
+    loadMat<CP>(A.mats + (size_t)matIdx * A.matStride + cc * 4, M);
     const uint8_t* t = A.states + (size_t)(tip ? -child - 1 : 0) * A.Ppad;
     const T* xg = static_cast<const T*>(A.partials) + (size_t)(tip ? 0 : child) * A.stride + off0;
 #pragma unroll
     for (int r = 0; r < R; ++r) {
         const int p = p0 + r * G;
         const bool live = ALIGNED || (catValid && p >= pBegin && p < pEnd);
-        double x[4], u[4], y[4];
+        double x[4], y[4];
         int s = 0;
         if (tip) {
             s = live ? (int)__ldg(t + p) : S;
@@ -90,12 +88,7 @@
         } else {
             x[0] = x[1] = x[2] = x[3] = 0.0;
         }
-#pragma unroll
-        for (int k = 0; k < 4; ++k)
-            u[k] = (Vi[4 * k] * x[0] + Vi[4 * k + 1] * x[1] + Vi[4 * k + 2] * x[2] + Vi[4 * k + 3] * x[3]) * e[k];
-#pragma unroll
-        for (int i = 0; i < 4; ++i)
-            y[i] = absBits(A.V[4 * i] * u[0] + A.V[4 * i + 1] * u[1] + A.V[4 * i + 2] * u[2] + A.V[4 * i + 3] * u[3]);
+        applyMat(M, x, y);
         if (tip && s >= S) {
 #pragma unroll
             for (int i = 0; i < 4; ++i) y[i] = (i < S) ? 1.0 : 0.0;
@@ -122,9 +115,6 @@
     double* tab1 = tipTab + (TIP == 2 ? ((threadIdx.x >> 5) * 2) * CP * 20 : 0);
     double* tab2 = tab1 + (TIP == 2 ? CP * 20 : 0);
 
-    double Vi[16];
-#pragma unroll
-    for (int q = 0; q < 16; ++q) asm volatile("mov.f64 %0, %1;" : "=d"(Vi[q]) : "d"(A.Vi[q]));
     Op4 cur = loadOp(A.ops + range.x);
     double d[R][4];
 #pragma unroll
@@ -147,15 +137,12 @@
                     if (ALIGNED || p0 + r * G < A.Ppad) prefetchL1(xg + (size_t)r * G * 4);
             }
         }
-        if (lane < 2) {
-            const int mi = lane == 0 ? cur.pfM1 : cur.pfM2;
-            if (mi >= 0) prefetchL1(A.evecs + (size_t)mi * CP * 4);
-        } else if (TIP != 0 && lane >= 8 && lane < 16) {
-            const int mi = lane < 12 ? cur.pfM1 : cur.pfM2;
+        if (lane < 8) {
+            const int mi = lane < 4 ? cur.pfM1 : cur.pfM2;
             if (mi >= 0) prefetchL1(A.mats + (size_t)mi * A.matStride + (lane & 3) * 4 * CP);
         }
-        childTermE<T, CP, R, ALIGNED, true, TIP>(A, Vi, cur.c1, cur.m1, (cur.pad_ & 2) != 0, cc, off0, p0, catValid, cur.pBegin, cur.pEnd, d, tab1);
-        childTermE<T, CP, R, ALIGNED, false, TIP>(A, Vi, cur.c2, cur.m2, false, cc, off0, p0, catValid, cur.pBegin, cur.pEnd, d, tab2);
+        childTermE<T, CP, R, ALIGNED, true, TIP>(A, cur.c1, cur.m1, (cur.pad_ & 2) != 0, cc, off0, p0, catValid, cur.pBegin, cur.pEnd, d, tab1);
+        childTermE<T, CP, R, ALIGNED, false, TIP>(A, cur.c2, cur.m2, false, cc, off0, p0, catValid, cur.pBegin, cur.pEnd, d, tab2);
         if (R != 1) nxt = loadOp(A.ops + min(k + 1, last));
         T* dg = static_cast<T*>(A.partials) + (size_t)cur.dest * A.stride + off0;
 #pragma unroll
@@ -211,9 +198,11 @@
 struct WarpStage {
     static constexpr int G = 32 / CP, NP = G * R, TABLES = VIRT ? 4 : 2;
     double mat[TABLES][5 * CP * 4];
-    double ev[2][CP * 4];
+    double pm[2][16 * CP];
     alignas(16) unsigned char st[TABLES][NP < 16 ? 16 : NP];
 };
+template <int CP, int R, bool VIRT>
+constexpr size_t stageBytes() { return 4 * 2 * sizeof(WarpStage<CP, R, VIRT>); }
 
 template <typename T, int CP, int R, bool VIRT>
 __device__ __forceinline__ void walk4pBody(const WalkArgs& A) {
@@ -222,7 +211,8 @@
     static_assert(NP % PIECE == 0 && (PIECE == 4 || PIECE == 8 || PIECE == 16), "state-byte staging");
     constexpr int TABLES = WarpStage<CP, R, VIRT>::TABLES;
     constexpr int RECQ = sizeof(Op4) / 16 + (VIRT ? 1 : 0);
-    __shared__ __align__(16) WarpStage<CP, R, VIRT> stages[4][2];
+    extern __shared__ __align__(16) unsigned char stageMem[];
+    auto stages = reinterpret_cast<WarpStage<CP, R, VIRT>(*)[2]>(stageMem);
     __shared__ __align__(16) Op4 rings[4][4];
     __shared__ __align__(16) int4 tipRings[4][VIRT ? 4 : 1];
     int lane;
@@ -275,7 +265,9 @@
                     stageBlock(sg.mat[ch], rcp);
                     stageBlock(sg.mat[TABLES - 2 + ch], rcp + 16 * CP);
                 }
-                if (lane < CP * 2) cpAsync16(&sg.ev[ch][2 * lane], A.evecs + (size_t)m * CP * 4 + 2 * lane);
+                const double* src = A.mats + (size_t)m * A.matStride;
+#pragma unroll
+                for (int q = lane; q < CP * 8; q += 32) cpAsync16(&sg.pm[ch][2 * q], src + 2 * q);
             }
         }
         constexpr int SL = NP / PIECE;
@@ -308,9 +300,6 @@
     asm volatile("cp.async.wait_group 0;" ::: "memory");
     __syncwarp();
 
-    double Vi[16];
-#pragma unroll
-    for (int q = 0; q < 16; ++q) asm volatile("mov.f64 %0, %1;" : "=d"(Vi[q]) : "d"(A.Vi[q]));
     double d[R][4];
 #pragma unroll
     for (int r = 0; r < R; ++r) d[r][0] = d[r][1] = d[r][2] = d[r][3] = 0.0;
@@ -341,15 +330,19 @@
                     else { d[r][0] *= lo.x; d[r][1] *= lo.y; d[r][2] *= hi.x; d[r][3] *= hi.y; }
                 }
             } else {
-                const double2* ep = reinterpret_cast<const double2*>(&sg.ev[ch][cc * 4]);
-                const double2 e01 = ep[0], e23 = ep[1];
-                const double e[4] = {e01.x, e01.y, e23.x, e23.y};
+                Mat4 M;
+#pragma unroll
+                for (int j = 0; j < 4; ++j) {
+                    const double2* row = reinterpret_cast<const double2*>(&sg.pm[ch][(j * CP + cc) * 4]);
+                    const double2 lo = row[0], hi = row[1];
+                    M.r[j][0] = lo.x; M.r[j][1] = lo.y; M.r[j][2] = hi.x; M.r[j][3] = hi.y;
+                }
                 const bool fromRegisters = ch == 0 && (cur.flags & 2) != 0;
                 const bool virt = VIRT && (cur.flags & (4 << ch)) != 0;
                 const T* xg = static_cast<const T*>(A.partials) + (size_t)child * A.stride + off0;
 #pragma unroll
                 for (int r = 0; r < R; ++r) {
-                    double x[4], u[4], y[4];
+                    double x[4], y[4];
                     if (fromRegisters) {
 #pragma unroll
                         for (int i = 0; i < 4; ++i) x[i] = d[r][i];
@@ -366,12 +359,7 @@
                     } else {
                         loadCell(xg + (size_t)r * G * 4, x);
                     }
-#pragma unroll
-                    for (int q = 0; q < 4; ++q)
-                        u[q] = (Vi[4 * q] * x[0] + Vi[4 * q + 1] * x[1] + Vi[4 * q + 2] * x[2] + Vi[4 * q + 3] * x[3]) * e[q];
-#pragma unroll
-                    for (int i = 0; i < 4; ++i)
-                        y[i] = absBits(A.V[4 * i] * u[0] + A.V[4 * i + 1] * u[1] + A.V[4 * i + 2] * u[2] + A.V[4 * i + 3] * u[3]);
+                    applyMat(M, x, y);
 #pragma unroll
                     for (int i = 0; i < 4; ++i) d[r][i] = ch == 0 ? y[i] : d[r][i] * y[i];
                 }
@@ -431,15 +419,19 @@
 
 template <typename T, int CP, int R, int MINB>
 cudaError_t launchP(Instance* in, const WalkArgs& A, dim3 grid) {
-    if constexpr (sizeof(T) == 4) k_walk4ps<CP, R, MINB><<<grid, 128, 0, in->stream>>>(A);
-    else k_walk4p<CP, R, MINB><<<grid, 128, 0, in->stream>>>(A);
+    constexpr size_t smem = stageBytes<CP, R, false>();
+    static_assert(smem <= 48 * 1024, "k_walk4p stages");
+    if constexpr (sizeof(T) == 4) k_walk4ps<CP, R, MINB><<<grid, 128, smem, in->stream>>>(A);
+    else k_walk4p<CP, R, MINB><<<grid, 128, smem, in->stream>>>(A);
     return cudaGetLastError();
 }
 
 template <typename T, int CP, int R>
 cudaError_t launchPV(Instance* in, const WalkArgs& A, dim3 grid) {
-    if constexpr (sizeof(T) == 4) k_walk4pvs<CP, R, 3><<<grid, 128, 0, in->stream>>>(A);
-    else k_walk4pv<CP, R, 3><<<grid, 128, 0, in->stream>>>(A);
+    constexpr size_t smem = stageBytes<CP, R, true>();
+    static_assert(smem <= 48 * 1024 || CP == 8, "only CP = 8 opts in to more shared memory (configureWalk4E)");
+    if constexpr (sizeof(T) == 4) k_walk4pvs<CP, R, 3><<<grid, 128, smem, in->stream>>>(A);
+    else k_walk4pv<CP, R, 3><<<grid, 128, smem, in->stream>>>(A);
     return cudaGetLastError();
 }
 
@@ -546,6 +538,9 @@
 template <typename T, int CP>
 cudaError_t launchCP(Instance* in, WalkArgs& A, int nSubs, int maxWindow, bool aligned, bool virt) {
     const int R = phaseR(in, nSubs, maxWindow);
+    if (in->debug)
+        fprintf(stderr, "[b200-beagle] walk: %s, R = %d, %d subtrees\n",
+                stagedWalk(in, R, aligned) ? (virt ? "k_walk4pv" : "k_walk4p") : "k_walk4e", R, nSubs);
     if (R == 1) return launchR<T, CP, 1>(in, A, nSubs, maxWindow, aligned, virt);
     if constexpr (CP == 4) {
         if (R == 8) return launchR<T, CP, 8>(in, A, nSubs, maxWindow, aligned, virt);
@@ -556,6 +551,19 @@
 
 }
 
+cudaError_t configureWalk4E(const Instance* in) {
+    if (in->matCP != 8) return cudaSuccess;
+    cudaError_t e = cudaSuccess;
+    auto optIn = [&](const void* kernel, size_t bytes) {
+        if (e == cudaSuccess) e = cudaFuncSetAttribute(kernel, cudaFuncAttributeMaxDynamicSharedMemorySize, (int)bytes);
+    };
+    optIn(reinterpret_cast<const void*>(k_walk4pv<8, 1, 3>), stageBytes<8, 1, true>());
+    optIn(reinterpret_cast<const void*>(k_walk4pv<8, 4, 3>), stageBytes<8, 4, true>());
+    optIn(reinterpret_cast<const void*>(k_walk4pvs<8, 1, 3>), stageBytes<8, 1, true>());
+    optIn(reinterpret_cast<const void*>(k_walk4pvs<8, 4, 3>), stageBytes<8, 4, true>());
+    return e;
+}
+
 bool walk4pServes(const Instance* in, int nSubs, int maxWindow) {
     if (in->matCP == 0) return false;
     const int R = phaseR(in, nSubs, maxWindow);
@@ -563,7 +571,7 @@
 }
 
 cudaError_t launchWalk4E(Instance* in, const Op4* dOps, const int4* dSubs, int nSubs, int maxWindow, bool aligned,
-                         const double* eigen, const int4* dVirtTips) {
+                         const int4* dVirtTips) {
     const bool virt = dVirtTips != nullptr;
     if (nSubs <= 0) return cudaSuccess;
     WalkArgs A;
@@ -571,11 +579,9 @@
     A.states = in->states8Base; A.mats = in->dMat; A.scale = in->dScale;
     A.S = in->S; A.C = in->C; A.Ppad = in->Ppad; A.logScalers = in->logScalers ? 1 : 0;
     A.matStride = in->matStride; A.matMmaOffset = 16 * in->matCP;
-    A.evecs = in->dEvec;
     A.recipes = in->dRecipe;
     A.virtTips = dVirtTips;
     if (virt && in->dRecipe == nullptr) return cudaErrorInvalidValue;
-    for (int q = 0; q < 16; ++q) { A.V[q] = eigen[q]; A.Vi[q] = eigen[16 + q]; }
     if (in->single) {
         switch (in->matCP) {
             case 1: return launchCP<float, 1>(in, A, nSubs, maxWindow, aligned, virt);
@@ -616,22 +622,4 @@
     return cudaGetLastError();
 }
 
-cudaError_t updateWalk4EGraph(cudaGraphExec_t exec, const std::vector<cudaGraphNode_t>& kernelNodes, const double* eigen) {
-    for (cudaGraphNode_t node : kernelNodes) {
-        cudaKernelNodeParams kp;
-        cudaError_t e = cudaGraphKernelNodeGetParams(node, &kp);
-        if (e != cudaSuccess) return e;
-        if (kp.func == reinterpret_cast<void*>(k_cherry_snapshot)) continue;
-        if (kp.kernelParams == nullptr || kp.kernelParams[0] == nullptr) return cudaErrorInvalidValue;
-        WalkArgs A = *static_cast<const WalkArgs*>(kp.kernelParams[0]);
-        for (int q = 0; q < 16; ++q) { A.V[q] = eigen[q]; A.Vi[q] = eigen[16 + q]; }
-        void* args[1] = {&A};
-        kp.kernelParams = args;
-        kp.extra = nullptr;
-        e = cudaGraphExecKernelNodeSetParams(exec, node, &kp);
-        if (e != cudaSuccess) return e;
-    }
-    return cudaSuccess;
-}
-
-}
+}
```

Result: faster. 2391 (median of 6 runs) (+6.3%).
